# sevagh/umx.cpp

Hardware: AMD Instinct MI355X
Metric: realtime-factor (audio-sec/wall-sec) UMX-L 4-stem, 60 s seg (higher is better)
Workload: dtype f32 (activations as 2 x fp16 planes of the power-of-two-scaled row, integer weights exact in fp16, f32 accumulate on the fp16 matrix cores; fp32-grade: 1.4-2.2x the error of an fp32 evaluation, profiles/r06_v2_accuracy_vs_float64.txt)

## Files before the change

include/umx_hip.h:

```cpp
#ifndef UMX_HIP_H
#define UMX_HIP_H

#include <stddef.h>
#include <stdint.h>

#ifdef __cplusplus
extern "C" {
#endif

#define UMX_OK 0
#define UMX_ERR_ARG 1
#define UMX_ERR_HIP 2
#define UMX_ERR_MODEL 3
#define UMX_ERR_TIMEOUT 4
#define UMX_ERR_NODEVICE 5

#define UMX_DTYPE_F32 0
#define UMX_DTYPE_U8 1
#define UMX_DTYPE_U16 2

#define UMX_FLAG_NO_WIENER 0x1
#define UMX_FLAG_WIENER_ITERS_MASK 0xF0000u
#define UMX_FLAG_WIENER_ITERS(n) ((((unsigned)(n)) & 0xFu) << 16)
#define UMX_FLAG_SKIP_TARGET(t) (0x100 << (t))
// ... 187 lines not shown
    int n_out;
    int hop;
} umx_loudness;
int umx_hip_separate_tracks_loudness(umx_hip_ctx *ctx, int n_tracks, const void *const *audio_host, const int *length, const int *rate,
                                     const int *shift_offset, int n_out, const float *gains, void *const *out_host, unsigned flags,
                                     const umx_sample_io *io, int clip_mode, umx_levels *levels, umx_loudness *loudness,
                                     double *const *hop_energy, void (*progress)(float, void *), void *progress_user);
typedef void (*umx_queue_loudness_fn)(void *user, const umx_queue_job *job, const umx_levels *levels, const umx_loudness *loudness,
                                      const double *hop_energy);
int umx_hip_separate_queue_loudness(umx_hip_ctx *ctx, umx_queue_next_fn next, umx_queue_loudness_fn done, void *user, int n_out,
                                    const float *gains, unsigned flags, const umx_sample_io *io, int clip_mode);
int umx_hip_kweight_hops_device(umx_hip_ctx *ctx, int n_buffers, const float *const *in_dev, int n, int rate, long long first_hop,
                                long long n_hops, double *E_dev, void *hip_stream);
int umx_hip_kweight_coeffs(int rate, double pb[3], double pa[3], double rb[3], double ra[3]);
int umx_hip_kweight_hops_host(const float *x, int n, int rate, long long first_hop, long long n_hops, double *E);
int umx_hip_loudness_gate(const double *E, long long hops, int hop, double *integrated, double *momentary_max, long long *blocks,
                          long long *gated);
#define UMX_TRUE_PEAK_OFF 0
#define UMX_TRUE_PEAK_MEASURE 1
#define UMX_TRUE_PEAK_RESCALE 2
typedef struct umx_true_peak
{
    float true_peak[4];
    int n_out;
    int factor;
} umx_true_peak;
int umx_hip_separate_tracks_true_peak(umx_hip_ctx *ctx, int n_tracks, const void *const *audio_host, const int *length, const int *rate,
                                      const int *shift_offset, int n_out, const float *gains, void *const *out_host, unsigned flags,
                                      const umx_sample_io *io, int clip_mode, umx_levels *levels, umx_loudness *loudness,
                                      double *const *hop_energy, int true_peak_mode, umx_true_peak *true_peak,
                                      void (*progress)(float, void *), void *progress_user);
typedef void (*umx_queue_true_peak_fn)(void *user, const umx_queue_job *job, const umx_levels *levels, const umx_loudness *loudness,
                                       const double *hop_energy, const umx_true_peak *true_peak);
int umx_hip_separate_queue_true_peak(umx_hip_ctx *ctx, umx_queue_next_fn next, umx_queue_true_peak_fn done, void *user, int n_out,
                                     const float *gains, unsigned flags, const umx_sample_io *io, int clip_mode, int true_peak_mode);
int umx_hip_true_peak_device(umx_hip_ctx *ctx, int n_buffers, const float *const *in_dev, int n, int rate, long long first_frame,
                             long long n_frames, unsigned *bits_dev, void *hip_stream);
int umx_hip_true_peak_taps(int rate, float taps[49], int *factor);
int umx_hip_true_peak_host(const float *x, int n, int rate, long long first_frame, long long n_frames, unsigned *bits);
int umx_hip_debug_resample_taps(int rate_in, int rate_out, float *taps, size_t cap, int *phases, int *taps_per_phase,
                                int *first_offset);

size_t umx_hip_stream_layer_floats(const umx_hip_ctx *ctx);
int umx_hip_stream_get_layer(umx_hip_ctx *ctx, int layer, float *host_dst);
int umx_hip_stream_set_layer(umx_hip_ctx *ctx, int layer, const float *host_src);
int umx_hip_segment_begin(umx_hip_ctx *ctx, const float *audio_host, int n, unsigned flags);
int umx_hip_segment_lstm_layer(umx_hip_ctx *ctx, int layer);
int umx_hip_segment_end(umx_hip_ctx *ctx, float *const out_host[4]);

int umx_hip_segment_masks_device(umx_hip_ctx *ctx);
int umx_hip_segment_residual_device(umx_hip_ctx *ctx);
float *umx_hip_target_mag_device(umx_hip_ctx *ctx, int target, size_t *floats);
int umx_hip_segment_finish_device(umx_hip_ctx *ctx, float *const out_dev[4]);
int umx_hip_segment_discard(umx_hip_ctx *ctx);
int umx_hip_gate_reserve(int device, int cus);
void *umx_hip_phase_stream(umx_hip_ctx *ctx);
float *umx_hip_stream_state_device(umx_hip_ctx *ctx);
int umx_hip_segment_begin_device(umx_hip_ctx *ctx, const float *audio_dev, int n, unsigned flags);
int umx_hip_segment_end_device(umx_hip_ctx *ctx, float *const out_dev[4]);
int umx_hip_weight_stems_device(umx_hip_ctx *ctx, float *const stems_dev[4], int n, void *hip_stream);
int umx_hip_track_accumulate_device(umx_hip_ctx *ctx, float *const track_dev[4], float *sum_weight_dev,
                                    const float *const weighted_dev[4], int offset, int n, void *hip_stream);
int umx_hip_track_normalise_device(umx_hip_ctx *ctx, float *const track_dev[4], const float *sum_weight_dev, int length,
                                   void *hip_stream);

int umx_hip_nb_frames(const umx_hip_ctx *ctx);
int umx_hip_segment_samples(const umx_hip_ctx *ctx);
int umx_hip_hidden(const umx_hip_ctx *ctx);

long umx_hip_read_tap(umx_hip_ctx *ctx, const char *what, int target, float *dst, size_t capacity_floats);

int umx_hip_stage_times(umx_hip_ctx *ctx, const char **names, float *ms, int cap);
int umx_hip_stage_times_slot(umx_hip_ctx *ctx, int slot_index, const char **names, float *ms, int cap);
int umx_hip_stage_kernel_times_slot(umx_hip_ctx *ctx, int slot_index, float *ms, int cap);
int umx_hip_lstm_was_persistent(const umx_hip_ctx *ctx);
const char *umx_hip_lstm_kernel_name(const umx_hip_ctx *ctx);
const char *umx_hip_gemm_kernel_name(const umx_hip_ctx *ctx, int mode);
int umx_hip_lstm_mode(umx_hip_ctx *ctx);
int umx_hip_debug_wiener_bins(int n, const float *X, const float *masks, const float *R, float max_abs, float *y);
int umx_hip_debug_gate_math(int n, const float *x, float *fn, int n_waves, const float *pre, const float *c, float *cell);
int umx_hip_debug_lstm_profile(umx_hip_ctx *ctx, unsigned long long *out48);
int umx_hip_debug_lstm_placement(umx_hip_ctx *ctx, unsigned long long *out, int n);
int umx_hip_debug_lds_guard(umx_hip_ctx *ctx, int launches, int rounds, unsigned *out2);
unsigned umx_hip_debug_f16_bits(float x);
int umx_hip_debug_quant_centre(float scale, float offset, float *o2);
int umx_hip_debug_quant_planes(const void *q, int elem_size, int n, float scale, float offset, unsigned short *hi, unsigned short *lo, float *o2);

#ifdef __cplusplus
}
#endif
#endif
```

umx.cpp_amd/__init__.py:

```python
import ctypes as C
import os
import subprocess
from pathlib import Path

import numpy as np

from . import ggml

HERE = Path(__file__).resolve().parent
ROOT = HERE.parent
NB, CROP, KX, NOUT, NFFT, HOP = 2049, 1487, 2976, 4098, 4096, 1024
SEGMENT_SAMPLES = 60 * 44100

UMX_OK, ERR_ARG, ERR_HIP, ERR_MODEL, ERR_TIMEOUT, ERR_NODEVICE = 0, 1, 2, 3, 4, 5
HOST_ERR_AUDIO = 12
DTYPE_F32, DTYPE_U8, DTYPE_U16 = 0, 1, 2
FLAG_NO_WIENER = 0x1
FLAG_SOFTMASK = 0x2
FLAG_LSTM_STEPWISE = 0x10
FLAG_DEBUG_TAPS = 0x20
FLAG_LSTM_FORCE_SAFE = 0x40
FLAG_LSTM_PROFILE = 0x80
FLAG_PRECISE_ACT = 0x1000
FLAG_DEBUG_LSTM_ABORT = 0x2000
# ... 138 lines not shown
        import torch
        torch.cuda.is_available()
    except Exception:
        pass
    path = Path(os.environ.get("UMX_HIP_LIB", HERE / "libumx_hip.so"))
    if not path.exists():
        raise ImportError(f"{path} is missing: run `python -c 'import __graft_entry__ as g; g.build()'` "
                          "(hipcc --offload-arch=gfx950). There is no CPU fallback.")
    lib = C.CDLL(str(path))
    lib.umx_hip_create.argtypes = [C.POINTER(C.c_void_p), C.c_int, C.c_int, C.c_int, C.POINTER(TensorView), C.c_int]
    lib.umx_hip_create_ex.argtypes = [C.POINTER(C.c_void_p), C.c_int, C.c_int, C.c_int, C.POINTER(TensorView), C.c_int,
                                      C.c_uint]
    lib.umx_hip_create_tracks.argtypes = [C.POINTER(C.c_void_p), C.c_int, C.c_int, C.c_int, C.POINTER(TensorView), C.c_int,
                                          C.c_uint, C.c_int]
    lib.umx_hip_n_tracks.argtypes = [C.c_void_p]
    lib.umx_hip_pipeline_depth.argtypes = [C.c_void_p]
    lib.umx_hip_lstm_is_batched.argtypes = [C.c_void_p]
    lib.umx_hip_debug_f16_bits.argtypes = [C.c_float]
    lib.umx_hip_debug_f16_bits.restype = C.c_uint
    lib.umx_hip_debug_quant_centre.argtypes = [C.c_float, C.c_float, C.POINTER(C.c_float)]
    lib.umx_hip_debug_quant_centre.restype = C.c_int
    lib.umx_hip_debug_quant_planes.argtypes = [C.c_void_p, C.c_int, C.c_int, C.c_float, C.c_float, C.c_void_p, C.c_void_p, C.POINTER(C.c_float)]
    lib.umx_hip_debug_quant_planes.restype = C.c_int
    lib.umx_hip_track_stream_reset.argtypes = [C.c_void_p, C.c_int]
    lib.umx_hip_track_stream_get.argtypes = [C.c_void_p, C.c_int, _fp]
    lib.umx_hip_track_stream_set.argtypes = [C.c_void_p, C.c_int, _fp]
    lib.umx_hip_infer_segment_async.argtypes = [C.c_void_p, C.c_void_p, C.c_int, C.POINTER(C.c_void_p), C.c_uint]
    lib.umx_hip_infer_batch.argtypes = [C.c_void_p, C.c_int, C.POINTER(C.c_void_p), C.POINTER(C.c_int), C.POINTER(C.c_void_p), C.c_uint]
    lib.umx_hip_infer_batch_async.argtypes = lib.umx_hip_infer_batch.argtypes
    lib.umx_hip_infer_batch_device.argtypes = lib.umx_hip_infer_batch.argtypes
    lib.umx_hip_order_after.argtypes = [C.c_void_p, C.c_void_p]
    lib.umx_hip_order_before.argtypes = [C.c_void_p, C.c_void_p]
    lib.umx_hip_weight_bytes.restype = C.c_size_t
    lib.umx_hip_weight_bytes.argtypes = [C.c_void_p]
    lib.umx_hip_destroy.argtypes = [C.c_void_p]
    lib.umx_hip_last_error.restype = C.c_char_p
    lib.umx_hip_last_error.argtypes = [C.c_void_p]
    lib.umx_hip_stream_floats.restype = C.c_size_t
    lib.umx_hip_stream_floats.argtypes = [C.c_void_p]
    lib.umx_hip_stream_reset.argtypes = [C.c_void_p]
    lib.umx_hip_stream_get.argtypes = [C.c_void_p, _fp]
    lib.umx_hip_stream_set.argtypes = [C.c_void_p, _fp]
    lib.umx_hip_infer_segment.argtypes = [C.c_void_p, _fp, C.c_int, C.POINTER(_fp), C.c_uint]
    lib.umx_hip_infer_segment_device.argtypes = [C.c_void_p, C.c_void_p, C.c_int, C.POINTER(C.c_void_p), C.c_uint]
    lib.umx_hip_sync.argtypes = [C.c_void_p]
    lib.umx_hip_stream_handle.restype = C.c_void_p
    lib.umx_hip_stream_handle.argtypes = [C.c_void_p]
    lib.umx_hip_nb_frames.argtypes = [C.c_void_p]
    lib.umx_hip_segment_samples.argtypes = [C.c_void_p]
    lib.umx_hip_hidden.argtypes = [C.c_void_p]
    lib.umx_hip_read_tap.restype = C.c_long
    lib.umx_hip_read_tap.argtypes = [C.c_void_p, C.c_char_p, C.c_int, _fp, C.c_size_t]
    lib.umx_hip_stage_times.argtypes = [C.c_void_p, C.POINTER(C.c_char_p), _fp, C.c_int]
    lib.umx_hip_stage_times_slot.argtypes = [C.c_void_p, C.c_int, C.POINTER(C.c_char_p), _fp, C.c_int]
    lib.umx_hip_stage_kernel_times_slot.argtypes = [C.c_void_p, C.c_int, _fp, C.c_int]
    lib.umx_hip_lstm_was_persistent.argtypes = [C.c_void_p]
    lib.umx_hip_lstm_mode.argtypes = [C.c_void_p]
    lib.umx_hip_debug_lstm_profile.argtypes = [C.c_void_p, C.POINTER(C.c_ulonglong)]
    lib.umx_hip_debug_wiener_bins.argtypes = [C.c_int, _fp, _fp, _fp, C.c_float, _fp]
    lib.umx_hip_debug_gate_math.argtypes = [C.c_int, _fp, _fp, C.c_int, _fp, _fp, _fp]
    lib.umx_hip_lstm_kernel_name.restype = C.c_char_p
    lib.umx_hip_lstm_kernel_name.argtypes = [C.c_void_p]
    lib.umx_hip_gemm_kernel_name.restype = C.c_char_p
    lib.umx_hip_gemm_kernel_name.argtypes = [C.c_void_p, C.c_int]
    lib.umx_hip_debug_lstm_placement.argtypes = [C.c_void_p, C.POINTER(C.c_ulonglong), C.c_int]
    lib.umx_hip_stream_layer_floats.restype = C.c_size_t
    lib.umx_hip_stream_layer_floats.argtypes = [C.c_void_p]
    lib.umx_hip_stream_get_layer.argtypes = [C.c_void_p, C.c_int, _fp]
    lib.umx_hip_stream_set_layer.argtypes = [C.c_void_p, C.c_int, _fp]
    lib.umx_hip_segment_begin.argtypes = [C.c_void_p, _fp, C.c_int, C.c_uint]
    lib.umx_hip_segment_lstm_layer.argtypes = [C.c_void_p, C.c_int]
    lib.umx_hip_segment_end.argtypes = [C.c_void_p, C.POINTER(_fp)]
    lib.umx_hip_segment_begin_device.argtypes = [C.c_void_p, C.c_void_p, C.c_int, C.c_uint]
    lib.umx_hip_segment_end_device.argtypes = [C.c_void_p, C.POINTER(C.c_void_p)]
    lib.umx_hip_segment_masks_device.argtypes = [C.c_void_p]
    lib.umx_hip_segment_residual_device.argtypes = [C.c_void_p]
    lib.umx_hip_residual_slot.argtypes = [C.c_uint]
    lib.umx_hip_segment_finish_device.argtypes = [C.c_void_p, C.POINTER(C.c_void_p)]
    lib.umx_hip_weight_stems_device.argtypes = [C.c_void_p, C.POINTER(C.c_void_p), C.c_int, C.c_void_p]
    lib.umx_hip_track_accumulate_device.argtypes = [C.c_void_p, C.POINTER(C.c_void_p), C.c_void_p, C.POINTER(C.c_void_p), C.c_int,
                                                    C.c_int, C.c_void_p]
    lib.umx_hip_track_normalise_device.argtypes = [C.c_void_p, C.POINTER(C.c_void_p), C.c_void_p, C.c_int, C.c_void_p]
    lib.umx_hip_debug_lds_guard.argtypes = [C.c_void_p, C.c_int, C.c_int, C.POINTER(C.c_uint)]
    lib.umx_hip_split_inference.argtypes = [C.c_void_p, _fp, C.c_int, C.POINTER(_fp), C.c_uint, C.c_void_p, C.c_void_p]
    lib.umx_hip_shift_inference.argtypes = [C.c_void_p, _fp, C.c_int, C.c_int, C.POINTER(_fp), C.c_uint, C.c_void_p,
                                            C.c_void_p]
    lib.umx_hip_resampled_length.restype = C.c_longlong
    lib.umx_hip_resampled_length.argtypes = [C.c_longlong, C.c_int, C.c_int]
    lib.umx_hip_resample_device.argtypes = [C.c_void_p, C.c_int, C.c_int, C.c_int, C.POINTER(C.c_void_p), C.c_int,
                                            C.POINTER(C.c_void_p), C.c_int, C.c_void_p]
    lib.umx_hip_resample_needs.restype = C.c_longlong
    lib.umx_hip_resample_needs.argtypes = [C.c_longlong, C.c_int, C.c_int, C.c_longlong]
    lib.umx_hip_resample_ready.restype = C.c_longlong
    lib.umx_hip_resample_ready.argtypes = [C.c_longlong, C.c_int, C.c_int, C.c_longlong, C.c_longlong]
    lib.umx_hip_resample_range_device.argtypes = [C.c_void_p, C.c_int, C.c_int, C.c_int, C.POINTER(C.c_void_p), C.c_int,
                                                  C.POINTER(C.c_void_p), C.c_int, C.c_int, C.c_int, C.c_void_p]
    lib.umx_hip_debug_resample_launches.argtypes = [C.c_void_p, C.POINTER(C.c_int), C.POINTER(C.c_int)]
    lib.umx_hip_shift_inference_rate.argtypes = [C.c_void_p, _fp, C.c_int, C.c_int, C.c_int, C.POINTER(_fp), C.c_uint, C.c_void_p,
                                                 C.c_void_p]
    lib.umx_hip_debug_resample_taps.argtypes = [C.c_int, C.c_int, _fp, C.c_size_t, C.POINTER(C.c_int), C.POINTER(C.c_int),
                                                C.POINTER(C.c_int)]
    lib.umx_hip_ensemble_offsets.argtypes = [C.c_int, C.c_int, C.POINTER(C.c_int)]
    lib.umx_hip_shift_ensemble.argtypes = [C.c_void_p, _fp, C.c_int, C.c_int, C.c_int, C.POINTER(C.c_int), C.POINTER(_fp), C.c_uint,
                                           C.c_void_p, C.c_void_p]
    lib.umx_hip_debug_shift_mean_ms.restype = C.c_float
    lib.umx_hip_debug_shift_mean_ms.argtypes = [C.c_void_p]
    lib.umx_hip_mix_columns.argtypes = [C.c_int, _fp]
    lib.umx_hip_shift_ensemble_mix.argtypes = [C.c_void_p, _fp, C.c_int, C.c_int, C.c_int, C.POINTER(C.c_int), C.c_int, _fp, C.POINTER(_fp),
                                               C.c_uint, C.c_void_p, C.c_void_p]
    lib.umx_hip_mix_stems_device.argtypes = [C.c_void_p, C.c_int, _fp, C.POINTER(C.c_void_p), C.c_void_p, C.c_int, C.POINTER(C.c_void_p),
                                             C.c_void_p]
    lib.umx_hip_queue_plan.argtypes = [C.c_int, C.c_int, C.POINTER(C.c_int), C.POINTER(C.c_int), C.POINTER(C.c_int), C.POINTER(C.c_int)]
    lib.umx_hip_debug_queue_calls.argtypes = [C.c_void_p]
    lib.umx_hip_pcm16_decode_device.argtypes = [C.c_void_p, C.c_void_p, C.c_int, C.c_void_p, C.c_void_p]
    lib.umx_hip_pcm16_encode_device.argtypes = [C.c_void_p, C.c_int, C.POINTER(C.c_void_p), C.c_int, C.c_longlong, C.POINTER(SampleIO),
                                                C.POINTER(C.c_void_p), C.c_void_p]
    lib.umx_hip_pcm16_decode_host.argtypes = [_i16p, C.c_longlong, _fp]
    lib.umx_hip_pcm16_encode_host.argtypes = [_fp, C.c_int, C.c_int, C.c_longlong, C.POINTER(SampleIO), _i16p]
    lib.umx_hip_pcm24_decode_device.argtypes = [C.c_void_p, C.c_void_p, C.c_int, C.c_void_p, C.c_void_p]
    lib.umx_hip_pcm24_encode_device.argtypes = [C.c_void_p, C.c_int, C.POINTER(C.c_void_p), C.c_int, C.c_longlong, C.POINTER(SampleIO),
                                                C.POINTER(C.c_void_p), C.c_void_p]
    lib.umx_hip_pcm24_encode_rescaled_device.argtypes = [C.c_void_p, C.c_int, C.POINTER(C.c_void_p), C.c_int, C.c_longlong, C.POINTER(SampleIO),
                                                         C.POINTER(C.c_void_p), C.c_void_p, C.c_void_p]
    lib.umx_hip_pcm24_decode_host.argtypes = [_u8p, C.c_longlong, _fp]
    lib.umx_hip_pcm24_encode_host.argtypes = [_fp, C.c_int, C.c_int, C.c_longlong, C.POINTER(SampleIO), _u8p]
    lib.umx_hip_levels_device.argtypes = [C.c_void_p, C.c_int, C.POINTER(C.c_void_p), C.c_int, C.c_longlong, C.POINTER(SampleIO), C.c_void_p,
                                          C.c_void_p]
    lib.umx_hip_pcm16_encode_rescaled_device.argtypes = [C.c_void_p, C.c_int, C.POINTER(C.c_void_p), C.c_int, C.c_longlong, C.POINTER(SampleIO),
                                                         C.POINTER(C.c_void_p), C.c_void_p, C.c_void_p]
    lib.umx_hip_rescale_device.argtypes = [C.c_void_p, C.c_int, C.POINTER(C.c_void_p), C.c_int, C.c_void_p, C.c_void_p]
    lib.umx_hip_levels_host.argtypes = [_fp, C.c_int, C.c_int, C.c_longlong, C.POINTER(SampleIO), C.c_float, C.POINTER(LevelsAcc)]
    lib.umx_hip_rescale_gain.argtypes = [_fp, C.c_int]
    lib.umx_hip_rescale_gain.restype = C.c_float
    lib.umx_hip_kweight_hops_device.argtypes = [C.c_void_p, C.c_int, C.POINTER(C.c_void_p), C.c_int, C.c_int, C.c_longlong, C.c_longlong,
                                                C.c_void_p, C.c_void_p]
    lib.umx_hip_kweight_coeffs.argtypes = [C.c_int, _dp, _dp, _dp, _dp]
    lib.umx_hip_kweight_hops_host.argtypes = [_fp, C.c_int, C.c_int, C.c_longlong, C.c_longlong, _dp]
    lib.umx_hip_loudness_gate.argtypes = [_dp, C.c_longlong, C.c_int, _dp, _dp, C.POINTER(C.c_longlong), C.POINTER(C.c_longlong)]
    lib.umx_hip_true_peak_device.argtypes = [C.c_void_p, C.c_int, C.POINTER(C.c_void_p), C.c_int, C.c_int, C.c_longlong, C.c_longlong,
                                             C.c_void_p, C.c_void_p]
    lib.umx_hip_true_peak_taps.argtypes = [C.c_int, _fp, C.POINTER(C.c_int)]
    lib.umx_hip_true_peak_host.argtypes = [_fp, C.c_int, C.c_int, C.c_longlong, C.c_longlong, _up]
    def tracks_args(ptr, rate=True, mix=True):
        return ([C.c_void_p, C.c_int, C.POINTER(ptr), C.POINTER(C.c_int)] + [C.POINTER(C.c_int)] * (2 if rate else 1)
                + ([C.c_int, _fp] if mix else []) + [C.POINTER(ptr), C.c_uint])

    progress = [C.c_void_p, C.c_void_p]
    wide = tracks_args(C.c_void_p) + [C.POINTER(SampleIO)]
    lib.umx_hip_separate_tracks.argtypes = tracks_args(_fp, rate=False, mix=False) + progress
    lib.umx_hip_separate_tracks_rate.argtypes = tracks_args(_fp, mix=False) + progress
    lib.umx_hip_separate_tracks_mix.argtypes = tracks_args(_fp) + progress
    lib.umx_hip_separate_tracks_io.argtypes = wide + progress
    lib.umx_hip_separate_tracks_levels.argtypes = wide + [C.c_int, C.POINTER(Levels)] + progress
    lib.umx_hip_separate_tracks_loudness.argtypes = wide + [C.c_int, C.POINTER(Levels), C.POINTER(Loudness), C.POINTER(C.c_void_p)] + progress
    lib.umx_hip_separate_tracks_true_peak.argtypes = (wide + [C.c_int, C.POINTER(Levels), C.POINTER(Loudness), C.POINTER(C.c_void_p), C.c_int,
                                                              C.POINTER(TruePeak)] + progress)

    def queue_args(done_fn):
        return [C.c_void_p, QUEUE_NEXT_FN, done_fn, C.c_void_p, C.c_int, _fp, C.c_uint]

    lib.umx_hip_separate_queue.argtypes = queue_args(QUEUE_DONE_FN)
    lib.umx_hip_separate_queue_io.argtypes = queue_args(QUEUE_DONE_FN) + [C.POINTER(SampleIO)]
    lib.umx_hip_separate_queue_levels.argtypes = queue_args(QUEUE_LEVELS_FN) + [C.POINTER(SampleIO), C.c_int]
    lib.umx_hip_separate_queue_loudness.argtypes = queue_args(QUEUE_LOUDNESS_FN) + [C.POINTER(SampleIO), C.c_int]
    lib.umx_hip_separate_queue_true_peak.argtypes = queue_args(QUEUE_TRUE_PEAK_FN) + [C.POINTER(SampleIO), C.c_int, C.c_int]
    _hip = lib
    return lib


CREATE_QUANTISED_RESIDENT = 0x1
CREATE_GEMM_F32 = 0x4
CREATE_DEQUANTISE_AT_LOAD = 0x8
CREATE_LSTM_BATCHED = 0x10
CREATE_U8_DEQUANT = 0x20
CREATE_GEMM_STAGED = 0x40
CREATE_GEMM_PLANES = 0x80
MAX_TRACKS = 64
MAX_SHIFTS = MAX_TRACKS
MAX_MIX_OUTPUTS, MIX_COLUMNS, MIX_COLUMN_MIXTURE = 4, 5, 4
MODEL_RATE = 44100
RESAMPLE_MIN_RATE, RESAMPLE_MAX_RATE = 8000, 192000

HIP_SYMBOLS = ["umx_hip_create", "umx_hip_create_ex", "umx_hip_create_tracks", "umx_hip_n_tracks", "umx_hip_lstm_is_batched",
               "umx_hip_track_stream_reset", "umx_hip_track_stream_get", "umx_hip_track_stream_set",
               "umx_hip_infer_segment_async", "umx_hip_infer_batch", "umx_hip_infer_batch_async",
               "umx_hip_infer_batch_device", "umx_hip_order_after", "umx_hip_order_before",
               "umx_hip_separate_tracks", "umx_hip_phase_stream", "umx_hip_stream_state_device", "umx_hip_segment_begin_device", "umx_hip_segment_end_device",
               "umx_hip_weight_stems_device", "umx_hip_track_accumulate_device", "umx_hip_track_normalise_device", "umx_hip_weight_bytes", "umx_hip_destroy", "umx_hip_last_error", "umx_hip_stream_floats",
               "umx_hip_stream_reset", "umx_hip_stream_get", "umx_hip_stream_set", "umx_hip_infer_segment",
               "umx_hip_infer_segment_device", "umx_hip_sync", "umx_hip_stream_handle", "umx_hip_nb_frames",
               "umx_hip_segment_samples", "umx_hip_hidden", "umx_hip_read_tap", "umx_hip_stage_times",
               "umx_hip_stage_times_slot", "umx_hip_stage_kernel_times_slot",
               "umx_hip_lstm_was_persistent", "umx_hip_lstm_mode", "umx_hip_lstm_kernel_name", "umx_hip_gemm_kernel_name", "umx_hip_debug_wiener_bins", "umx_hip_debug_gate_math", "umx_hip_debug_lstm_profile", "umx_hip_debug_lstm_placement",
               "umx_hip_stream_layer_floats", "umx_hip_stream_get_layer", "umx_hip_stream_set_layer",
               "umx_hip_segment_begin", "umx_hip_segment_lstm_layer", "umx_hip_segment_end",
               "umx_hip_split_inference", "umx_hip_shift_inference", "umx_hip_debug_lds_guard", "umx_hip_debug_f16_bits", "umx_hip_debug_quant_centre", "umx_hip_debug_quant_planes",
               "umx_hip_segment_masks_device", "umx_hip_target_mag_device", "umx_hip_segment_finish_device", "umx_hip_gate_reserve", "umx_hip_segment_discard", "umx_hip_pipeline_depth",
               "umx_hip_resampled_length", "umx_hip_resample_device", "umx_hip_shift_inference_rate", "umx_hip_separate_tracks_rate",
               "umx_hip_debug_resample_taps", "umx_hip_residual_slot", "umx_hip_segment_residual_device",
               "umx_hip_ensemble_offsets", "umx_hip_shift_ensemble", "umx_hip_debug_shift_mean_ms",
               "umx_hip_mix_columns", "umx_hip_separate_tracks_mix", "umx_hip_shift_ensemble_mix", "umx_hip_mix_stems_device",
               "umx_hip_separate_queue", "umx_hip_queue_plan", "umx_hip_debug_queue_calls",
               "umx_hip_separate_tracks_io", "umx_hip_separate_queue_io", "umx_hip_pcm16_decode_device", "umx_hip_pcm16_encode_device",
               "umx_hip_pcm16_decode_host", "umx_hip_pcm16_encode_host",
               "umx_hip_separate_tracks_levels", "umx_hip_separate_queue_levels", "umx_hip_levels_device",
               "umx_hip_pcm16_encode_rescaled_device", "umx_hip_rescale_device", "umx_hip_levels_host", "umx_hip_rescale_gain",
               "umx_hip_separate_tracks_loudness", "umx_hip_separate_queue_loudness", "umx_hip_kweight_hops_device",
               "umx_hip_kweight_coeffs", "umx_hip_kweight_hops_host", "umx_hip_loudness_gate",
               "umx_hip_resample_needs", "umx_hip_resample_ready", "umx_hip_resample_range_device", "umx_hip_debug_resample_launches",
               "umx_hip_pcm24_decode_device", "umx_hip_pcm24_encode_device", "umx_hip_pcm24_encode_rescaled_device",
               "umx_hip_pcm24_decode_host", "umx_hip_pcm24_encode_host",
               "umx_hip_separate_tracks_true_peak", "umx_hip_separate_queue_true_peak", "umx_hip_true_peak_device",
               "umx_hip_true_peak_taps", "umx_hip_true_peak_host"]


def sample_io(in_format=SAMPLE_F32, out_format=SAMPLE_F32, dither_seed=None):
    return SampleIO(int(in_format), int(out_format), 0 if dither_seed is None else 1, 0 if dither_seed is None else int(dither_seed) & 0xFFFFFFFF)


def pcm16_decode_host(q):
    q = np.ascontiguousarray(q, np.int16)
    x = np.empty(q.shape, np.float32)
    rc = hip_lib().umx_hip_pcm16_decode_host(q.ctypes.data_as(_i16p), q.size, x.ctypes.data_as(_fp))
    if rc != UMX_OK:
        raise UmxError(rc, "umx_hip_pcm16_decode_host")
    return x


def _encode_host(fmt, x, buffer, first_frame, dither_seed):
    a = np.ascontiguousarray(np.asarray(x, np.float32).T)
    q, qp, out_format = {16: (np.empty(a.shape, np.int16), _i16p, SAMPLE_S16), 24: (np.empty(6 * a.shape[0], np.uint8), _u8p, SAMPLE_S24)}[fmt]
    io = sample_io(SAMPLE_F32, out_format, dither_seed)
    name = f"umx_hip_pcm{fmt}_encode_host"
    rc = getattr(hip_lib(), name)(a.ctypes.data_as(_fp), a.shape[0], int(buffer), int(first_frame), C.byref(io), q.ctypes.data_as(qp))
    if rc != UMX_OK:
        raise UmxError(rc, name)
    return q


def pcm16_encode_host(x, buffer=0, first_frame=0, dither_seed=None):
    return np.ascontiguousarray(_encode_host(16, x, buffer, first_frame, dither_seed).T)


def pcm24_pack(q):
    a = np.ascontiguousarray(np.asarray(q, np.int32).T)
    if a.ndim != 2 or a.shape[1] != 2:
        raise ValueError("pcm24_pack: need a (2, L) array")
    if a.size and (a.min() < -8388608 or a.max() > 8388607):
        raise ValueError("pcm24_pack: codes outside -8388608 .. 8388607")
    return np.ascontiguousarray(a.astype("<i4").view(np.uint8).reshape(-1, 4)[:, :3]).ravel()


def pcm24_unpack(b):
    b = np.ascontiguousarray(b, np.uint8).ravel()
    if b.size % 6:
        raise ValueError("pcm24_unpack: need a multiple of 6 bytes")
    w = np.zeros((b.size // 3, 4), np.uint8)
    w[:, 1:] = b.reshape(-1, 3)
    return np.ascontiguousarray((w.view("<i4").ravel().astype(np.int32) >> 8).reshape(-1, 2).T)


def pcm24_decode_host(q):
    q = np.ascontiguousarray(q, np.int32)
    b = np.ascontiguousarray(q.ravel().astype("<i4").view(np.uint8).reshape(-1, 4)[:, :3]).ravel()
    x = np.empty(q.shape, np.float32)
    rc = hip_lib().umx_hip_pcm24_decode_host(b.ctypes.data_as(_u8p), q.size, x.ctypes.data_as(_fp))
    if rc != UMX_OK:
        raise UmxError(rc, "umx_hip_pcm24_decode_host")
    return x


def pcm24_encode_host(x, buffer=0, first_frame=0, dither_seed=None):
    return pcm24_unpack(_encode_host(24, x, buffer, first_frame, dither_seed))


def levels_host(x, buffer=0, first_frame=0, io=None, clip_divisor=1.0, acc=None):
    a = np.ascontiguousarray(np.asarray(x, np.float32).T)
    acc = LevelsAcc() if acc is None else acc
    rc = hip_lib().umx_hip_levels_host(a.ctypes.data_as(_fp), a.shape[0], int(buffer), int(first_frame), None if io is None else C.byref(io),
# ... 647 lines not shown
            a = np.ascontiguousarray(wv.T).ravel()
            o = [np.empty(2 * wv.shape[1], np.float32) for _ in range(4)]
            keep.append((a, o))
            aud[i], ns[i] = a.ctypes.data, wv.shape[1]
            for t in range(4):
                outs[4 * i + t] = o[t].ctypes.data
        self._check(self.lib.umx_hip_infer_batch(self.h, nb, aud, ns, outs, flags))
        res, k = [], 0
        for wv in waves:
            if wv is None:
                res.append(None)
                continue
            n = keep[k][0].size // 2
            res.append([np.ascontiguousarray(o.reshape(n, 2).T) for o in keep[k][1]])
            k += 1
        return res

    def infer_batch_ptrs(self, audio_ptrs, ns, out_ptrs, flags=0, where="device"):
        nb = len(audio_ptrs)
        aud = (C.c_void_p * nb)(*[p or None for p in audio_ptrs])
        n_ = (C.c_int * nb)(*ns)
        outs = (C.c_void_p * (4 * nb))(*[p or None for p in out_ptrs])
        fn = self.lib.umx_hip_infer_batch_device if where == "device" else self.lib.umx_hip_infer_batch_async
        self._check(fn(self.h, nb, aud, n_, outs, flags))

    def infer_segment_device(self, audio_ptr, n, out_ptrs, flags=0):
        arr = (C.c_void_p * 4)(*out_ptrs)
        self._check(self.lib.umx_hip_infer_segment_device(self.h, C.c_void_p(audio_ptr), n, arr, flags))

    def sync(self):
        self._check(self.lib.umx_hip_sync(self.h))

    def last_error(self):
        return self.lib.umx_hip_last_error(self.h).decode()

    def lstm_was_persistent(self):
        return bool(self.lib.umx_hip_lstm_was_persistent(self.h))

    def lstm_mode(self):
        return self.lib.umx_hip_lstm_mode(self.h)

    def lstm_profile(self):
        buf = (C.c_ulonglong * 48)()
        self._check(self.lib.umx_hip_debug_lstm_profile(self.h, buf))
        a = np.array(buf[:], dtype=np.uint64).reshape(3, 2, 8)
        return a

    def gemm_kernel_name(self, mode):
        return self.lib.umx_hip_gemm_kernel_name(self.h, mode).decode()

    def lstm_kernel_name(self):
        return self.lib.umx_hip_lstm_kernel_name(self.h).decode()

    def lstm_placement(self, n=256):
        buf = (C.c_ulonglong * n)()
        self._check(self.lib.umx_hip_debug_lstm_placement(self.h, buf, n))
        a = np.array(buf[:], dtype=np.uint64)
        return [(int(v >> 48) & 15, int(v >> 40) & 255, int(v >> 32) & 255, int(v) & 0xffffffff) for v in a]

    def tap(self, what, target=0):
        n = self.lib.umx_hip_read_tap(self.h, what.encode(), target, None, 0)
        if n < 0:
            raise UmxError(ERR_ARG, f"tap {what!r} unavailable ({n})")
        buf = np.empty(n, np.float32)
        got = self.lib.umx_hip_read_tap(self.h, what.encode(), target, buf.ctypes.data_as(_fp), n)
        if got != n:
            raise UmxError(ERR_HIP, f"tap {what!r} failed ({got})")
        T, H = self.T, self.hidden
        what = what.split("@")[0].split("#")[0]
        if what in ("lstm_l0", "lstm_l1"):
            return buf.reshape(T, H)
        if what == "proj":
            return buf.reshape(T, 4 * H)
        if what in ("spec", "y"):
            return buf.view(np.complex64).reshape(2, T, NB)
        if what in ("mix_mag", "target_mag"):
            return buf.reshape(2, T, NB)
        if what == "x":
            return buf.reshape(T, KX)
        if what in ("fc1", "lstm", "fc2"):
            return buf.reshape(T, H)
        if what == "mask":
            return buf.reshape(T, NOUT)
        return buf

    def stage_times(self, slot=None):
        names = (C.c_char_p * 32)()
        ms = (C.c_float * 32)()
        if slot is None:
            n = self.lib.umx_hip_stage_times(self.h, names, ms, 32)
        else:
            n = self.lib.umx_hip_stage_times_slot(self.h, slot, names, ms, 32)
        return {names[i].decode(): float(ms[i]) for i in range(n)}

    def stage_kernel_times(self, slot=None):
        names = (C.c_char_p * 32)()
        ms = (C.c_float * 32)()
        n = self.lib.umx_hip_stage_times_slot(self.h, 0, names, (C.c_float * 32)(), 32)
        m = self.lib.umx_hip_stage_kernel_times_slot(self.h, -1 if slot is None else slot, ms, 32)
        return {names[i].decode(): float(ms[i]) for i in range(min(n, m))}


HOST_SYMBOLS = ["umx_model_load", "umx_model_free", "umx_model_hidden", "umx_model_n_tensors", "umx_model_views",
                "umx_model_data_bytes", "umx_model_load_progress", "umx_model_dequantize", "umx_wav_load",
                "umx_wav_free", "umx_wav_write_f32", "umx_wav_load_rate", "umx_wav_write_f32_rate",
                "umx_wav_load_pcm16", "umx_wav_free_pcm16", "umx_wav_write_pcm16_rate",
                "umx_wav_load_pcm24", "umx_wav_free_pcm24", "umx_wav_write_pcm24_rate", "umx_split_inference", "umx_shift_inference",
                "umx_segment_plan", "umx_transition_weight", "umx_split_inference_carry", "umx_split_inference_targets", "umx_mix_parse"]

SEGMENT_FN = C.CFUNCTYPE(C.c_int, C.c_void_p, _fp, C.c_int, C.POINTER(_fp))
RESET_FN = C.CFUNCTYPE(C.c_int, C.c_void_p)
PROGRESS_FN = C.CFUNCTYPE(None, C.c_float, C.c_void_p)


PH_BEGIN_FN = C.CFUNCTYPE(C.c_int, C.c_void_p, _fp, C.c_int)
PH_LAYER_FN = C.CFUNCTYPE(C.c_int, C.c_void_p, C.c_int)
PH_END_FN = C.CFUNCTYPE(C.c_int, C.c_void_p, C.POINTER(_fp))
PH_STATE_FN = C.CFUNCTYPE(C.c_int, C.c_void_p, C.c_int, _fp)
P2P_FN = C.CFUNCTYPE(C.c_int, C.c_void_p, _fp, C.c_size_t, C.c_int)


class PhasedBackend(C.Structure):
    _fields_ = [("begin", PH_BEGIN_FN), ("layer", PH_LAYER_FN), ("end", PH_END_FN), ("get_layer", PH_STATE_FN),
                ("set_layer", PH_STATE_FN), ("layer_floats", C.c_size_t), ("user", C.c_void_p)]


TG_BEGIN_FN = C.CFUNCTYPE(C.c_int, C.c_void_p, _fp, C.c_int, C.c_uint)
TG_STATE_FN = C.CFUNCTYPE(C.c_int, C.c_void_p, C.c_int, C.c_int, _fp)
TG_VOID_FN = C.CFUNCTYPE(C.c_int, C.c_void_p)
TG_MAG_FN = C.CFUNCTYPE(C.c_int, C.c_void_p, C.c_int, _fp)


class TargetBackend(C.Structure):
    _fields_ = [("begin", TG_BEGIN_FN), ("layer", PH_LAYER_FN), ("get_state", TG_STATE_FN), ("set_state", TG_STATE_FN),
                ("masks", TG_VOID_FN), ("get_mag", TG_MAG_FN), ("set_mag", TG_MAG_FN), ("finish", PH_END_FN), ("discard", TG_VOID_FN),
                ("target_layer_floats", C.c_size_t), ("mag_floats", C.c_size_t), ("user", C.c_void_p)]


class P2P(C.Structure):
    _fields_ = [("send", P2P_FN), ("recv", P2P_FN), ("user", C.c_void_p)]


class Backend(C.Structure):
    _fields_ = [("segment", SEGMENT_FN), ("reset", RESET_FN), ("user", C.c_void_p)]


_host = None


def host_lib():
    global _host
    if _host is not None:
        return _host
    path = HERE / "libumx_host.so"
    if not path.exists():
        raise ImportError(f"{path} is missing: run __graft_entry__.build()")
    lib = C.CDLL(str(path))
    lib.umx_model_load.argtypes = [C.c_char_p, C.POINTER(C.c_void_p), C.c_char_p]
    lib.umx_model_free.argtypes = [C.c_void_p]
    lib.umx_model_hidden.argtypes = [C.c_void_p]
    lib.umx_model_n_tensors.argtypes = [C.c_void_p]
    lib.umx_model_views.restype = C.POINTER(TensorView)
    lib.umx_model_views.argtypes = [C.c_void_p]
    lib.umx_model_data_bytes.restype = C.c_size_t
    lib.umx_model_data_bytes.argtypes = [C.c_void_p]
    lib.umx_model_load_progress.restype = C.c_float
    lib.umx_model_load_progress.argtypes = [C.c_void_p]
# ... 312 lines not shown
```

umx.cpp_amd/csrc/engine.hip:

```cpp
#include "../../include/umx_hip.h"
#include <chrono>
#include <dlfcn.h>

#include <algorithm>
#include <numeric>
#include <cmath>
#include <cstdio>
#include <cstdlib>
#include <cstring>
#include <map>
#include <mutex>
#include <string>
#include <vector>

#include "common.h"
#include "gemm_bf16x3.h"
#include "gemm_planes.h"
#include "gemm_planes_pp.h"
#include "gemm_planes_ps.h"
#include "lstm_kernels.h"
#include "lstm_batch.h"
#include "lstm_batch8.h"
#include "track_kernels.h"
#include "resample.h"
#include "stft_kernels.h"
#include "wiener_kernels.h"
#include "wiener_istft.h"
#include "wiener_em.h"
#include "residual_mask.h"
#include "softmask.h"
#include "shift_mean.h"
#include "stem_mix.h"
#include "sample_format.h"
#include "pcm16.h"
#include "pcm24.h"
#include "levels.h"
#include "loudness.h"
#include "true_peak.h"
#include "gate_debug.h"

using namespace umx;

#define UMX_HIP_CHECK_CTX(ctx_, expr)                                                                                \
    do                                                                                                               \
    {                                                                                                                \
        hipError_t _e = (expr);                                                                                      \
        if (_e != hipSuccess)                                                                                        \
        {                                                                                                            \
            (ctx_)->set_error(std::string(#expr) + ": " + hipGetErrorString(_e));                                    \
            return UMX_ERR_HIP;                                                                                      \
        }                                                                                                            \
    } while (0)

namespace
{
std::string g_create_error = "";

enum { W_FC1 = 0, W_IH0, W_IH1, W_IH2, W_FC2, W_FC3, W_COUNT };
inline int gemm_weight(int mode, int layer) { return mode == G_FC1 ? W_FC1 : mode == G_IH ? W_IH0 + layer : mode == G_FC2 ? W_FC2 : W_FC3; }

struct GemmWeight
{
    const void *p = nullptr;
    int form = 0;
    float s[2] = {1.f, 1.f}, o[2] = {0.f, 0.f};
    float c[2] = {128.f, 128.f}, o2[2] = {0.f, 0.f};
};

struct TargetBufs
{
    GemmWeight w[W_COUNT];
    float *in_scale = nullptr, *in_mean = nullptr, *bn1[4] = {};
    float *ih_b[3] = {};
    float *bn2[4] = {};
    float *bn3[4] = {}, *out_scale = nullptr, *out_mean = nullptr;
};

struct TargetAct
{
    float *cat = nullptr, *la = nullptr, *lb = nullptr, *P = nullptr, *a2 = nullptr,
          *mag = nullptr;
    unsigned short *xs_p = nullptr, *cat_p = nullptr, *la_p = nullptr, *lb_p = nullptr, *a2_p = nullptr;
    float *rs_xs = nullptr, *rs_catL = nullptr, *rs_catR = nullptr, *rs_la = nullptr, *rs_lb = nullptr, *rs_a2 = nullptr;
    float *rsc_xs = nullptr, *rsc_a2 = nullptr;
};

enum
{
    ST_STFT = 0,
    ST_FC1,
    ST_IH0,
    ST_LSTM0,
    ST_IH1,
    ST_LSTM1,
    ST_IH2,
    ST_LSTM2,
    ST_FC2,
    ST_FC3,
    ST_WIENER,
    ST_ISTFT,
    ST_OLA,
    ST_COUNT
};
enum { SP_XS = 0, SP_CATL, SP_LA, SP_LB, SP_CATR, SP_A2 };
const char *kStageNames[ST_COUNT] = {"stft",  "fc1", "lstm_ih0", "lstm_rec0", "lstm_ih1", "lstm_rec1", "lstm_ih2",
                                     "lstm_rec2", "fc2", "fc3_mask", "wiener",  "istft",    "ola"};

namespace
{
struct RoctxApi
{
    int (*push)(const char *) = nullptr;
    int (*pop)() = nullptr;
    char names[ST_COUNT][40];
    RoctxApi()
    {
        for (int i = 0; i < ST_COUNT; ++i)
            snprintf(names[i], sizeof names[i], "umx:%s", kStageNames[i]);
        const char *want = getenv("UMX_ROCTX");
        const bool force = want && atoi(want) != 0;
        for (const char *lib : {"librocprofiler-sdk-roctx.so", "libroctx64.so"})
            if (void *h = dlopen(lib, force ? (RTLD_NOW | RTLD_LOCAL) : (RTLD_NOW | RTLD_NOLOAD)))
            {
                push = reinterpret_cast<int (*)(const char *)>(dlsym(h, "roctxRangePushA"));
                pop = reinterpret_cast<int (*)()>(dlsym(h, "roctxRangePop"));
                if (push && pop)
                    return;
                push = nullptr;
                pop = nullptr;
            }
    }
};
thread_local bool t_stage_range_open = false;
inline void stage_range(int stage)
{
    static const RoctxApi api;
    if (!api.push)
        return;
    if (t_stage_range_open)
        api.pop();
    t_stage_range_open = stage >= 0 && stage < ST_COUNT;
    if (t_stage_range_open)
        api.push(api.names[stage]);
}
struct StageRangeCloser
{
    ~StageRangeCloser() { stage_range(-1); }
};
}

struct Lane
{
    TargetAct ta[4];
    float2 *spec = nullptr, *y = nullptr, *frames = nullptr;
    float *x = nullptr, *wpart = nullptr, *Rc = nullptr;
    unsigned *maxabs = nullptr;
};

// ... 577 lines not shown
```

umx.cpp_amd/csrc/engine_cabi.h:

```cpp
template <class From, class To>
static bool device_buffers(umx_hip_ctx *ctx, const char *what, int n_buffers, From *const *bufs, int n, long long first_frame, To *p[4])
{
    if (n_buffers < 1 || n_buffers > 4 || !bufs || n < 1 || first_frame < 0)
    {
        ctx->set_error(std::string(what) + ": need 1 .. 4 buffers, n >= 1 and first_frame >= 0");
        return false;
    }
    for (int b = 0; b < n_buffers; ++b)
    {
        if (!bufs[b])
        {
            ctx->set_error(std::string(what) + ": null buffer");
            return false;
        }
        p[b] = reinterpret_cast<To *>(bufs[b]);
    }
    return true;
}

struct DitherArg
{
    bool on;
    uint32_t seed;
};
// ... 902 lines not shown

__global__ void debug_wiener_bins_kernel(int n, const float *X, const float *masks, const float *R, float max_abs, float *y)
{
    const int b = blockIdx.x * blockDim.x + threadIdx.x;
    if (b >= n)
        return;
    const float2 X0 = make_float2(X[b * 4 + 0], X[b * 4 + 1]), X1 = make_float2(X[b * 4 + 2], X[b * 4 + 3]);
    const float h0 = mix_magnitude(X0), h1 = mix_magnitude(X1);
    float m0[4], m1[4];
    float4 rc[4];
    for (int s = 0; s < 4; ++s)
    {
        m0[s] = masks[(b * 4 + s) * 2 + 0] * h0;
        m1[s] = masks[(b * 4 + s) * 2 + 1] * h1;
        rc[s] = make_float4(R[(b * 4 + s) * 4 + 0], R[(b * 4 + s) * 4 + 1], R[(b * 4 + s) * 4 + 2], R[(b * 4 + s) * 4 + 3]);
    }
    WienerBin wb;
    wiener_bin_setup(X0, X1, m0, m1, rc, max_abs, 1.0f / max_abs, wb);
    for (int s = 0; s < 4; ++s)
    {
        float2 o[2];
        wiener_bin_apply(wb, s, rc[s], max_abs, o);
        y[((b * 4 + s) * 2 + 0) * 2 + 0] = o[0].x;
        y[((b * 4 + s) * 2 + 0) * 2 + 1] = o[0].y;
        y[((b * 4 + s) * 2 + 1) * 2 + 0] = o[1].x;
        y[((b * 4 + s) * 2 + 1) * 2 + 1] = o[1].y;
    }
}
int umx_hip_debug_wiener_bins(int n, const float *X, const float *masks, const float *R, float max_abs, float *y)
{
    if (n < 1 || !X || !masks || !R || !y || !(max_abs >= 1.0f))
        return UMX_ERR_ARG;
    float *d = nullptr;
    const size_t nx = (size_t)n * 4, nm = (size_t)n * 8, nr = (size_t)n * 16, ny = (size_t)n * 16;
    if (hipMalloc(reinterpret_cast<void **>(&d), (nx + nm + nr + ny) * sizeof(float)) != hipSuccess)
        return UMX_ERR_HIP;
    bool ok = hipMemcpy(d, X, nx * 4, hipMemcpyHostToDevice) == hipSuccess && hipMemcpy(d + nx, masks, nm * 4, hipMemcpyHostToDevice) == hipSuccess &&
              hipMemcpy(d + nx + nm, R, nr * 4, hipMemcpyHostToDevice) == hipSuccess;
    if (ok)
    {
        hipLaunchKernelGGL(debug_wiener_bins_kernel, dim3((n + 63) / 64), dim3(64), 0, nullptr, n, d, d + nx, d + nx + nm, max_abs, d + nx + nm + nr);
        ok = hipDeviceSynchronize() == hipSuccess && hipMemcpy(y, d + nx + nm + nr, ny * 4, hipMemcpyDeviceToHost) == hipSuccess;
    }
    (void)hipFree(d);
    return ok ? UMX_OK : UMX_ERR_HIP;
}

int umx_hip_debug_gate_math(int n, const float *x, float *fn, int n_waves, const float *pre, const float *c, float *cell)
{
    if (n < 0 || n_waves < 0 || (n > 0 && (!x || !fn)) || (n_waves > 0 && (!pre || !c || !cell)) || n > (1 << 24) || n_waves > (1 << 16))
        return UMX_ERR_ARG;
    const size_t nx = (size_t)n, nf = (size_t)5 * n, np_ = (size_t)n_waves * 64, nc = (size_t)n_waves * 16, no = (size_t)n_waves * 128;
    if (nx + np_ == 0)
        return UMX_OK;
    float *d = nullptr;
    if (hipMalloc(reinterpret_cast<void **>(&d), (nx + nf + np_ + nc + no) * sizeof(float)) != hipSuccess)
        return UMX_ERR_HIP;
    float *dx = d, *dfn = dx + nx, *dpre = dfn + nf, *dc = dpre + np_, *dcell = dc + nc;
    bool ok = true;
    if (n > 0)
    {
        ok = hipMemcpy(dx, x, nx * 4, hipMemcpyHostToDevice) == hipSuccess;
        if (ok)
            hipLaunchKernelGGL(debug_gate_fn_kernel, dim3((n + 255) / 256), dim3(256), 0, nullptr, n, dx, dfn);
    }
    if (ok && n_waves > 0)
    {
        ok = hipMemcpy(dpre, pre, np_ * 4, hipMemcpyHostToDevice) == hipSuccess && hipMemcpy(dc, c, nc * 4, hipMemcpyHostToDevice) == hipSuccess;
        if (ok)
        {
            hipLaunchKernelGGL(debug_gate_cell_kernel<0>, dim3(n_waves), dim3(64), 0, nullptr, dpre, dc, dcell);
            hipLaunchKernelGGL(debug_gate_cell_kernel<1>, dim3(n_waves), dim3(64), 0, nullptr, dpre, dc, dcell + nc * 2);
            hipLaunchKernelGGL(debug_gate_cell_kernel<2>, dim3(n_waves), dim3(64), 0, nullptr, dpre, dc, dcell + nc * 4);
            hipLaunchKernelGGL(debug_gate_cell_kernel<3>, dim3(n_waves), dim3(64), 0, nullptr, dpre, dc, dcell + nc * 6);
        }
    }
    ok = ok && hipDeviceSynchronize() == hipSuccess;
    if (ok && n > 0)
        ok = hipMemcpy(fn, dfn, nf * 4, hipMemcpyDeviceToHost) == hipSuccess;
    if (ok && n_waves > 0)
        ok = hipMemcpy(cell, dcell, no * 4, hipMemcpyDeviceToHost) == hipSuccess;
    (void)hipFree(d);
    return ok ? UMX_OK : UMX_ERR_HIP;
}

int umx_hip_debug_lds_guard(umx_hip_ctx *ctx, int launches, int rounds, unsigned *out2)
{
    static hipStream_t gs = nullptr;
    static unsigned *errs = nullptr;
    if (!ctx)
        return UMX_ERR_ARG;
    if (!gs)
    {
        if (hipStreamCreateWithFlags(&gs, hipStreamNonBlocking) != hipSuccess || hipMalloc(&errs, 8) != hipSuccess)
            return UMX_ERR_HIP;
        (void)hipMemset(errs, 0, 8);
    }
    for (int i = 0; i < launches; ++i)
        hipLaunchKernelGGL(lds_guard_kernel, dim3(512), dim3(256), 0, gs, errs, rounds);
    if (launches == 0 && out2)
    {
        (void)hipStreamSynchronize(gs);
        (void)hipMemcpy(out2, errs, 8, hipMemcpyDeviceToHost);
        (void)hipMemset(errs, 0, 8);
    }
    return UMX_OK;
}

int umx_hip_segment_begin(umx_hip_ctx *ctx, const float *audio_host, int n, unsigned flags)
{
    return ctx ? ctx->phase_begin(audio_host, n, flags) : UMX_ERR_ARG;
}
int umx_hip_segment_lstm_layer(umx_hip_ctx *ctx, int layer) { return ctx ? ctx->phase_layer(layer) : UMX_ERR_ARG; }
int umx_hip_segment_end(umx_hip_ctx *ctx, float *const out_host[4]) { return ctx ? ctx->phase_end(out_host) : UMX_ERR_ARG; }

void *umx_hip_phase_stream(umx_hip_ctx *ctx) { return ctx ? (void *)ctx->slot[0].stream : nullptr; }
float *umx_hip_stream_state_device(umx_hip_ctx *ctx) { return ctx ? ctx->state : nullptr; }
int umx_hip_segment_begin_device(umx_hip_ctx *ctx, const float *audio_dev, int n, unsigned flags)
{
    return ctx ? ctx->phase_begin_device(audio_dev, n, flags) : UMX_ERR_ARG;
}
int umx_hip_segment_end_device(umx_hip_ctx *ctx, float *const out_dev[4]) { return ctx ? ctx->phase_end_device(out_dev) : UMX_ERR_ARG; }
int umx_hip_segment_masks_device(umx_hip_ctx *ctx) { return ctx ? ctx->phase_masks() : UMX_ERR_ARG; }
int umx_hip_segment_residual_device(umx_hip_ctx *ctx) { return ctx ? ctx->phase_residual() : UMX_ERR_ARG; }
int umx_hip_residual_slot(unsigned flags) { return residual_slot_of(flags); }
int umx_hip_segment_discard(umx_hip_ctx *ctx)
{
    if (!ctx)
        return UMX_ERR_ARG;
    stage_range(-1);
    ctx->ph_next = -1;
    ctx->cur = 0;
    ctx->clear_used();
    return UMX_OK;
}
int umx_hip_segment_finish_device(umx_hip_ctx *ctx, float *const out_dev[4]) { return ctx ? ctx->phase_finish_device(out_dev) : UMX_ERR_ARG; }
float *umx_hip_target_mag_device(umx_hip_ctx *ctx, int target, size_t *floats)
{
    if (!ctx || target < 0 || target > 3)
        return nullptr;
    if (floats)
        *floats = (size_t)2 * ctx->T * MAGP;
    return ctx->slot[0].lane[0].ta[target].mag;
}
int umx_hip_gate_reserve(int device, int cus)
{
    if (device < 0)
        return UMX_ERR_ARG;
    LstmGate &g = g_gate[device & 15];
    std::lock_guard<std::mutex> lock(g.m);
    if (cus > 0)
        g.reservations.push_back(cus);
    else if (cus < 0)
    {
        auto it = std::find(g.reservations.begin(), g.reservations.end(), -cus);
        if (it == g.reservations.end())
            return UMX_ERR_ARG;
        g.reservations.erase(it);
    }
    else
        g.reservations.clear();
    g.reserved = 2 * std::accumulate(g.reservations.begin(), g.reservations.end(), 0);
    return UMX_OK;
}

static Stems4 stems4(float *const p[4])
// ... 197 lines not shown
    umx_hip_ctx::DeferredDownload d;
    d.valid = true;
    d.si = si;
    d.nb = n_tracks;
    for (int ln = 0; ln < n_tracks; ++ln)
    {
        d.n[ln] = ain[ln] ? n[ln] : 0;
        for (int s = 0; s < 4; ++s)
            d.host[4 * ln + s] = out_host[4 * ln + s];
    }
    return ctx->queue_download(d, ctx->copy_stream);
}

int umx_hip_infer_batch(umx_hip_ctx *ctx, int n_tracks, const float *const *audio_host, const int *n, float *const *out_host,
                        unsigned flags)
{
    if (int rc = umx_hip_infer_batch_async(ctx, n_tracks, audio_host, n, out_host, flags))
        return rc;
    return umx_hip_sync(ctx);
}

int umx_hip_infer_segment_async(umx_hip_ctx *ctx, const float *audio_host, int n, float *const out_host[4], unsigned flags)
{
    if (!ctx || !audio_host || !out_host)
    {
        if (ctx)
            ctx->set_error("infer_segment: bad arguments");
        return UMX_ERR_ARG;
    }
    return umx_hip_infer_batch_async(ctx, 1, &audio_host, &n, out_host, flags);
}

int umx_hip_infer_segment(umx_hip_ctx *ctx, const float *audio_host, int n, float *const out_host[4], unsigned flags)
{
    if (int rc = umx_hip_infer_segment_async(ctx, audio_host, n, out_host, flags))
        return rc;
    return umx_hip_sync(ctx);
}

void *umx_hip_stream_handle(umx_hip_ctx *ctx) { return ctx ? (void *)ctx->slot[ctx->cur].stream : nullptr; }
int umx_hip_nb_frames(const umx_hip_ctx *ctx) { return ctx ? ctx->T : 0; }
int umx_hip_segment_samples(const umx_hip_ctx *ctx) { return ctx ? ctx->N : 0; }
int umx_hip_hidden(const umx_hip_ctx *ctx) { return ctx ? ctx->H : 0; }

long umx_hip_read_tap(umx_hip_ctx *ctx, const char *what, int target, float *dst, size_t cap)
{
    if (!ctx || !what || target < 0 || target > 3)
        return -1;
    std::string w = what;
    const int T = ctx->T, H = ctx->H;
    int which = ctx->cur, lane = 0;
    {
        const size_t hash = w.find('#');
        if (hash != std::string::npos)
        {
            lane = atoi(w.c_str() + hash + 1);
            const size_t at = w.find('@', hash);
            w = w.substr(0, hash) + (at == std::string::npos ? "" : w.substr(at));
            if (lane < 0 || lane >= ctx->B)
                return -1;
        }
    }
    if (w.size() > 2 && w[w.size() - 2] == '@')
    {
        which = w.back() - '0';
        w = w.substr(0, w.size() - 2);
        if (which < 0 || which >= ctx->nslots)
            return -1;
    }
    const Lane &sl = ctx->slot[which].lane[lane];
    const void *src = nullptr;
    size_t nfl = 0, src_ld = 0, rows = 0, cols = 0;
    int computed = 0;
    if (w == "spec") { src = sl.spec; nfl = (size_t)2 * 2 * T * NBINS; }
    else if (w == "mix_mag") { src = sl.spec; computed = 1; nfl = (size_t)2 * T * NBINS; }
    else if (w == "x") { src = sl.x; nfl = (size_t)T * KX; }
    else if (w == "fc1") { src = sl.ta[target].cat; rows = T; cols = H; src_ld = 2 * H; nfl = rows * cols; }
    else if (w == "lstm") { src = sl.ta[target].cat + H; rows = T; cols = H; src_ld = 2 * H; nfl = rows * cols; }
    else if (w == "lstm_l0") { src = sl.ta[target].la; nfl = (size_t)T * H; }
    else if (w == "lstm_l1") { src = sl.ta[target].lb; nfl = (size_t)T * H; }
    else if (w == "proj") { src = sl.ta[target].P; nfl = (size_t)T * 4 * H; }
    else if (w == "fc2") { src = sl.ta[target].a2; nfl = (size_t)T * H; }
    else if (w == "mask") { src = sl.ta[target].mag; computed = 3; nfl = (size_t)T * NOUT; }
    else if (w == "target_mag") { src = sl.ta[target].mag; computed = 2; nfl = (size_t)2 * T * NBINS; }
    else if (w == "y") { src = sl.y + (size_t)target * 2 * T * NBINS; nfl = (size_t)2 * 2 * T * NBINS; }
    else if (w == "max_abs") { src = sl.maxabs; nfl = 1; }
    else return -1;
    if ((w == "lstm" && !ctx->slot[which].lstm_rows_f32[2]) || (w == "lstm_l0" && !ctx->slot[which].lstm_rows_f32[0]) ||
        (w == "lstm_l1" && !ctx->slot[which].lstm_rows_f32[1]))
        return -2;
    if (!src)
        return -2;
    if (!dst)
        return (long)nfl;
    if (cap < nfl)
        return -3;
    if (ctx->sync_all() != UMX_OK)
        return -4;
    if (computed)
    {
        if (!ctx->tap_tmp && ctx->dalloc(&ctx->tap_tmp, (size_t)2 * T * NBINS) != UMX_OK)
            return -4;
        const unsigned blocks = (unsigned)((nfl + 255) / 256);
        if (computed == 1)
            hipLaunchKernelGGL(tap_mix_mag_kernel, dim3(blocks), dim3(256), 0, nullptr, sl.spec, nfl, ctx->tap_tmp);
        else if (computed == 2)
            hipLaunchKernelGGL(tap_target_mag_kernel, dim3(blocks), dim3(256), 0, nullptr, sl.spec, sl.ta[target].mag, nfl, ctx->tap_tmp);
        else
            hipLaunchKernelGGL(tap_mask_kernel, dim3(blocks), dim3(256), 0, nullptr, sl.ta[target].mag, T, ctx->tap_tmp);
        if (hipDeviceSynchronize() != hipSuccess)
            return -4;
        src = ctx->tap_tmp;
    }
    hipError_t e;
    if (rows)
        e = hipMemcpy2D(dst, cols * sizeof(float), src, src_ld * sizeof(float), cols * sizeof(float), rows,
                        hipMemcpyDeviceToHost);
    else
        e = hipMemcpy(dst, src, nfl * sizeof(float), hipMemcpyDeviceToHost);
    if (e != hipSuccess)
    {
        ctx->set_error(hipGetErrorString(e));
        return -4;
    }
    if (w == "max_abs")
    {
        unsigned bits;
        memcpy(&bits, dst, 4);
        float m;
        memcpy(&m, &bits, 4);
        dst[0] = std::max(1.0f, m / WIENER_SCALE);
    }
    return (long)nfl;
}

int umx_hip_stage_times_slot(umx_hip_ctx *ctx, int slot_index, const char **names, float *ms, int cap);
int umx_hip_stage_times(umx_hip_ctx *ctx, const char **names, float *ms, int cap)
{
    return ctx ? umx_hip_stage_times_slot(ctx, ctx->cur, names, ms, cap) : 0;
}

int umx_hip_stage_times_slot(umx_hip_ctx *ctx, int slot_index, const char **names, float *ms, int cap)
{
    if (!ctx || slot_index < 0 || slot_index >= ctx->nslots)
        return 0;
    Slot &sl = ctx->slot[slot_index];
    if (!sl.have_times || ctx->sync_all() != UMX_OK)
        return 0;
    int n = std::min(cap, (int)ST_COUNT);
    for (int i = 0; i < n; ++i)
    {
        float t = 0.f;
        (void)hipEventElapsedTime(&t, sl.ev[i], sl.ev[i + 1]);
        if (names)
            names[i] = kStageNames[i];
        if (ms)
            ms[i] = t;
    }
    return ST_COUNT;
}

int umx_hip_stage_kernel_times_slot(umx_hip_ctx *ctx, int slot_index, float *ms, int cap)
{
    if (ctx && slot_index < 0)
        slot_index = ctx->cur;
    if (!ctx || slot_index >= ctx->nslots)
// ... 54 lines not shown
```

umx.cpp_amd/csrc/engine_init.h:

```cpp
namespace
{
bool dequant(const umx_tensor_view &tv, size_t expect, std::vector<float> &out)
{
    size_t nel = 1;
    for (int i = 0; i < tv.n_dims; ++i)
        nel *= (size_t)tv.ne[i];
    if (nel != expect)
        return false;
    out.resize(nel);
    if (tv.dtype == UMX_DTYPE_F32)
        memcpy(out.data(), tv.data, nel * sizeof(float));
    else if (tv.dtype == UMX_DTYPE_U8)
    {
        const uint8_t *q = static_cast<const uint8_t *>(tv.data);
        for (size_t i = 0; i < nel; ++i)
            out[i] = (float)q[i] * tv.scale + tv.offset;
    }
    else if (tv.dtype == UMX_DTYPE_U16)
    {
        const uint16_t *q = static_cast<const uint16_t *>(tv.data);
        for (size_t i = 0; i < nel; ++i)
            out[i] = (float)q[i] * tv.scale + tv.offset;
    }
    else
// ... 37 lines not shown
    device = device_;
    UMX_HIP_CHECK(hipSetDevice(device));
    H = hidden;
    Hl = H / 2;
    S = Hl / LSTM_UNITS_PER_WG;
    N = segment_samples;
    T = N / HOP + 1;
    Tp = T;
    nbatch = (T + WIENER_BATCH - 1) / WIENER_BATCH;

    std::map<std::string, const umx_tensor_view *> idx[4];
    for (int i = 0; i < n_tensors; ++i)
    {
        if (tensors[i].target < 0 || tensors[i].target > 3 || !tensors[i].name || !tensors[i].data)
        {
            set_error("tensor view with bad target / name / data");
            return UMX_ERR_MODEL;
        }
        idx[tensors[i].target][tensors[i].name] = &tensors[i];
    }
    auto get = [&](int tg, const std::string &name, size_t expect, std::vector<float> &out) -> bool {
        auto it = idx[tg].find(name);
        if (it == idx[tg].end())
        {
            set_error("missing tensor '" + name + "' for target " + std::to_string(tg));
            return false;
        }
        if (!dequant(*it->second, expect, out))
        {
            set_error("tensor '" + name + "' has wrong size in model (target " + std::to_string(tg) + ")");
            return false;
        }
        return true;
    };

    const bool keepq = !(create_flags & UMX_CREATE_DEQUANTISE_AT_LOAD);
    auto view = [&](int tg, const std::string &name) -> const umx_tensor_view * {
        auto it = idx[tg].find(name);
        return it == idx[tg].end() ? nullptr : it->second;
    };
    auto all_q = [&](const std::string &name, int dtype, size_t expect) {
        for (int tg = 0; tg < 4; ++tg)
        {
            const umx_tensor_view *tv = view(tg, name);
            size_t n = 1;
            for (int i = 0; tv && i < tv->n_dims; ++i)
                n *= (size_t)tv->ne[i];
            if (!keepq || !tv || tv->dtype != dtype || n != expect)
                return false;
        }
        return true;
    };

    if (create_flags & UMX_CREATE_GEMM_F32)
    {
        set_error("UMX_CREATE_GEMM_F32: the fp32-MFMA GEMM flavour was removed in round 3 (slower and, against float64, less accurate "
                  "than the split-operand kernels: profiles/r02_accuracy_vs_float64.txt)");
        return UMX_ERR_ARG;
    }
    if (const char *e = getenv("UMX_GEMM_PP"))
        env_gemm_pp = atoi(e);
    if (const char *e = getenv("UMX_GEMM_PS"))
        env_gemm_ps = atoi(e);
    if (const char *e = getenv("UMX_LSTM8_POLL_DELAY"))
        lstm8_poll_delay = atoi(e);
    if (const char *e = getenv("UMX_LSTM8_PAIRED"))
        env_lstm8_paired = atoi(e) != 0;
    if (const char *e = getenv("UMX_LSTM8_MIN_LANES"))
        env_lstm8_min = atoi(e);
    if (const char *e = getenv("UMX_LSTM_POLL_DELAY"))
        lstm_poll_delay = atoi(e);
    wiener_fused = lstm_batched;
    if (const char *e = getenv("UMX_WIENER"))
        wiener_fused = std::string(e) == "fused";
    gemm_planes = (create_flags & UMX_CREATE_GEMM_PLANES) || (lstm_batched && !(create_flags & UMX_CREATE_GEMM_STAGED));
    Tp = gemm_planes ? std::max(T, 256) : round_up(T, 128);

    const int G = 4 * Hl;
    std::vector<int> gate_row(G);
    for (int sl = 0; sl < S; ++sl)
        for (int g = 0; g < 4; ++g)
            for (int u = 0; u < 16; ++u)
                gate_row[g * Hl + sl * 16 + u] = sl * 64 + u * 4 + g;
    std::vector<int> fc3_row(NOUT);
    for (int r = 0; r < NOUT; ++r)
        fc3_row[r] = r / NBINS * MAGP + r % NBINS;
    struct WeightDesc
    {
        std::string name[2];
        int nsrc, rows, cols, dst_rows, cols_pad;
        const std::vector<int> *dst_row;
        int dtype;
    };
    WeightDesc wd[W_COUNT];
    wd[W_FC1] = {{"fc1.weight"}, 1, H, NIN, H, KX, nullptr, UMX_DTYPE_U8};
    for (int l = 0; l < 3; ++l)
        wd[W_IH0 + l] = {{"lstm.weight_ih_l" + std::to_string(l), "lstm.weight_ih_l" + std::to_string(l) + "_reverse"}, 2, G, H, G, H, &gate_row,
                         UMX_DTYPE_U8};
    wd[W_FC2] = {{"fc2.weight"}, 1, H, 2 * H, H, 2 * H, nullptr, UMX_DTYPE_U16};
    wd[W_FC3] = {{"fc3.weight"}, 1, NOUT, H, NOUT_PAD, H, &fc3_row, UMX_DTYPE_U16};
    auto upload_weight = [&](GemmWeight &w, const void *host, size_t bytes) -> int {
        unsigned char *p = nullptr;
        if (int rc = dalloc(&p, bytes, false))
            return rc;
        UMX_HIP_CHECK(hipMemcpy(p, host, bytes, hipMemcpyHostToDevice));
        w.p = p;
        weight_bytes += bytes;
        return UMX_OK;
    };
    const bool exact_ok = keepq && !u8_dequant;
    auto load_weight = [&](int tg, const WeightDesc &d, GemmWeight &w) -> int {
        const size_t n = (size_t)d.nsrc * d.dst_rows * d.cols_pad;
        auto dst = [&](int s, int r) { return ((size_t)s * d.dst_rows + (d.dst_row ? (*d.dst_row)[r] : r)) * d.cols_pad; };
        bool q = true;
        for (int s = 0; s < d.nsrc; ++s)
            q = q && all_q(d.name[s], d.dtype, (size_t)d.rows * d.cols);
        std::vector<unsigned short> planes;
        if (q && (!gemm_planes || exact_ok))
        {
            const size_t esz = d.dtype == UMX_DTYPE_U8 ? 1 : 2;
            if (gemm_planes)
            {
                w.form = (int)esz;
                planes.assign(w.form * n, 0);
                for (int s = 0; s < d.nsrc; ++s)
                {
                    const umx_tensor_view *tv = view(tg, d.name[s]);
                    unsigned short *hi = planes.data() + (size_t)s * d.dst_rows * d.cols_pad;
                    const QuantCentre qc = quant_planes(tv->data, (int)esz, d.rows, d.cols, d.dst_row ? d.dst_row->data() : nullptr, (size_t)d.cols_pad,
                                                        tv->scale, tv->offset, hi, esz == 2 ? hi + n : nullptr);
                    w.s[s] = tv->scale;
                    w.o[s] = qc.o2;
                }
                return upload_weight(w, planes.data(), planes.size() * sizeof(unsigned short));
            }
            std::vector<unsigned char> qh(n * esz, 0);
            for (int s = 0; s < d.nsrc; ++s)
            {
                const umx_tensor_view *tv = view(tg, d.name[s]);
                for (int r = 0; r < d.rows; ++r)
                    memcpy(&qh[dst(s, r) * esz], static_cast<const unsigned char *>(tv->data) + (size_t)r * d.cols * esz, (size_t)d.cols * esz);
                w.s[s] = tv->scale;
                w.o[s] = tv->offset;
            }
            for (int s = 0; s < d.nsrc && esz == 1; ++s)
            {
                const QuantCentre qc = quant_centre(w.s[s], w.o[s]);
                w.c[s] = (float)qc.c;
                w.o2[s] = qc.o2;
            }
            w.form = esz == 1 ? BQ_U8 : BQ_U16;
            return upload_weight(w, qh.data(), qh.size());
        }
        std::vector<float> f(n, 0.f), v;
        if (gemm_planes)
            planes.assign(2 * n, 0);
        for (int s = 0; s < d.nsrc; ++s)
        {
            if (!get(tg, d.name[s], (size_t)d.rows * d.cols, v))
                return UMX_ERR_MODEL;
            for (int r = 0; r < d.rows; ++r)
                memcpy(&f[dst(s, r)], &v[(size_t)r * d.cols], sizeof(float) * d.cols);
            if (gemm_planes)
            {
                float mx = 0.f, scale = 1.f;
                for (float x : v)
                    if (std::isfinite(x))
                        mx = std::max(mx, std::fabs(x));
                if (mx > 0.f)
                {
                    int x;
                    (void)std::frexp(mx, &x);
                    const int e = std::min(std::max(GP_SPLIT_FIXED_EXP + 1 - x, -100), 100);
                    scale = std::ldexp(1.0f, e);
                    w.s[s] = std::ldexp(1.0f, -e);
                }
                const size_t b0 = (size_t)s * d.dst_rows * d.cols_pad;
                for (size_t i = b0; i < b0 + (size_t)d.dst_rows * d.cols_pad; ++i)
                    f16_split(f[i] * scale, &planes[i], &planes[n + i]);
            }
        }
        if (gemm_planes)
            w.form = 2;
        else
        {
            w.form = BQ_F32;
            planes.resize(3 * n);
            for (size_t i = 0; i < n; ++i)
                split3_host(f[i], planes[i], planes[n + i], planes[2 * n + i]);
        }
        return upload_weight(w, planes.data(), planes.size() * sizeof(unsigned short));
    };

    std::vector<float> whh_h[3], bhh_h[3];
    std::vector<unsigned char> whh_qh[3];
    bool whh_all_u8 = true;
    for (int l = 0; l < 3; ++l)
        for (int dir = 0; dir < 2; ++dir)
            whh_all_u8 = whh_all_u8 && all_q("lstm.weight_hh_l" + std::to_string(l) + (dir ? "_reverse" : ""), UMX_DTYPE_U8, (size_t)G * Hl);
    if (whh_all_u8)
        for (int l = 0; l < 3; ++l)
            whh_qh[l].assign((size_t)8 * S * Hl * 64, 0);
    for (int l = 0; l < 3; ++l)
    {
        whh_h[l].assign((size_t)8 * S * Hl * 64, 0.f);
        bhh_h[l].assign((size_t)8 * S * 64, 0.f);
    }
    for (int tg = 0; tg < 4; ++tg)
    {
        TargetBufs &b = tb[tg];
        std::vector<float> v, w;
        if (!get(tg, "input_scale", CROP, v))
            return UMX_ERR_MODEL;
        w.assign(KX, 0.f);
        for (int k = 0; k < NIN; ++k)
            w[k] = v[k % CROP];
        if (int rc = upload(&b.in_scale, w))
            return rc;
        if (!get(tg, "input_mean", CROP, v))
            return UMX_ERR_MODEL;
        w.assign(KX, 0.f);
        for (int k = 0; k < NIN; ++k)
            w[k] = v[k % CROP];
        if (int rc = upload(&b.in_mean, w))
            return rc;
        if (!get(tg, "output_scale", NBINS, v))
            return UMX_ERR_MODEL;
        w.assign(NOUT_PAD, 0.f);
        for (int c = 0; c < 2; ++c)
            for (int k = 0; k < NBINS; ++k)
                w[c * MAGP + k] = v[k];
        if (int rc = upload(&b.out_scale, w))
            return rc;
        if (!get(tg, "output_mean", NBINS, v))
            return UMX_ERR_MODEL;
        w.assign(NOUT_PAD, 0.f);
        for (int c = 0; c < 2; ++c)
            for (int k = 0; k < NBINS; ++k)
                w[c * MAGP + k] = v[k];
        if (int rc = upload(&b.out_mean, w))
            return rc;
        if (int rc = load_weight(tg, wd[W_FC1], b.w[W_FC1]))
            return rc;
        const char *bnn[4] = {"running_mean", "running_var", "weight", "bias"};
        for (int k = 0; k < 4; ++k)
        {
            if (!get(tg, std::string("bn1.") + bnn[k], H, v))
                return UMX_ERR_MODEL;
            if (int rc = upload(&b.bn1[k], v))
                return rc;
            if (!get(tg, std::string("bn2.") + bnn[k], H, v))
                return UMX_ERR_MODEL;
            if (int rc = upload(&b.bn2[k], v))
                return rc;
            if (!get(tg, std::string("bn3.") + bnn[k], NOUT, v))
                return UMX_ERR_MODEL;
            w.assign(NOUT_PAD, k == 1 ? 1.f : 0.f);
            for (int c = 0; c < 2; ++c)
                memcpy(&w[c * MAGP], &v[c * NBINS], sizeof(float) * NBINS);
            if (int rc = upload(&b.bn3[k], w))
                return rc;
        }
        if (int rc = load_weight(tg, wd[W_FC2], b.w[W_FC2]))
            return rc;
        if (int rc = load_weight(tg, wd[W_FC3], b.w[W_FC3]))
            return rc;
        for (int l = 0; l < 3; ++l)
        {
            if (int rc = load_weight(tg, wd[W_IH0 + l], b.w[W_IH0 + l]))
                return rc;
            std::vector<float> ihb((size_t)2 * G);
            for (int dir = 0; dir < 2; ++dir)
            {
                const std::string sfx = "_l" + std::to_string(l) + (dir ? "_reverse" : "");
                std::vector<float> whhv, bih, bhhv;
                if ((!whh_all_u8 && !get(tg, "lstm.weight_hh" + sfx, (size_t)G * Hl, whhv)) ||
                    !get(tg, "lstm.bias_ih" + sfx, G, bih) || !get(tg, "lstm.bias_hh" + sfx, G, bhhv))
                    return UMX_ERR_MODEL;
                const int chain = tg * 2 + dir;
                const umx_tensor_view *hhv = view(tg, "lstm.weight_hh" + sfx);
                const unsigned char *hhq = whh_all_u8 ? static_cast<const unsigned char *>(hhv->data) : nullptr;
                if (whh_all_u8)
                {
                    whh_s[l][chain] = hhv->scale;
                    whh_o[l][chain] = hhv->offset;
                }
                for (int row = 0; row < G; ++row)
                {
                    const int sl = gate_row[row] / 64, col = gate_row[row] % 64;
                    ihb[(size_t)dir * G + gate_row[row]] = bih[row];
                    bhh_h[l][((size_t)chain * S + sl) * 64 + col] = bhhv[row];
                    for (int k = 0; k < Hl; ++k)
                    {
                        const size_t di = (((size_t)chain * S + sl) * Hl + k) * 64 + col;
                        if (whh_all_u8)
                            whh_qh[l][di] = hhq[(size_t)row * Hl + k];
                        else
                            whh_h[l][di] = whhv[(size_t)row * Hl + k];
                    }
                }
            }
            if (int rc = upload(&b.ih_b[l], ihb))
                return rc;
        }
    }
    for (int l = 0; l < 3; ++l)
    {
        if (whh_all_u8)
        {
            if (int rc = upload(&whh_q[l], whh_qh[l]))
                return rc;
            weight_bytes += whh_qh[l].size();
        }
        else
        {
            if (int rc = upload(&whh[l], whh_h[l]))
                return rc;
            weight_bytes += whh_h[l].size() * sizeof(float);
        }
        if (int rc = upload(&bhh[l], bhh_h[l]))
            return rc;
    }
    {
        std::vector<float> w(NFFT);
        static const float PI = 3.14159265359F;
        const float floatN = (float)(NFFT + 1);
        for (int n = 0; n < NFFT; ++n)
            w[n] = 0.5F * (1.0F - cosf(2.0F * PI * (float)n / (floatN - 1)));
        if (int rc = upload(&window, w))
            return rc;
        const size_t total = (size_t)NFFT + (size_t)HOP * (T - 1);
        std::vector<float> nwh(total, 0.f);
        for (int i = 0; i < T; ++i)
        {
            const size_t s0 = (size_t)i * HOP;
            for (size_t j = s0; j < std::min(total, s0 + NFFT); ++j)
                nwh[j] += w[j - s0] * w[j - s0];
        }
        if (int rc = upload(&nw, nwh))
            return rc;
        std::vector<float2> t1(256), t2(4096);
        for (int r = 0; r < 16; ++r)
            for (int k = 0; k < 16; ++k)
            {
// ... 254 lines not shown
```

umx.cpp_amd/csrc/engine_stages.h:

```cpp
void umx_hip_ctx::launch_gemm(Lane &sl, hipStream_t st, int mode, int layer, const int *active, int nact, bool dbg)
{
    GemmArgs g;
    memset(&g, 0, sizeof g);
    g.M = Tp;
    g.T = T;
    int bq = BQ_F32;
    for (int i = 0; i < nact; ++i)
    {
        const TargetBufs &b = tb[active[i]];
        const TargetAct &c = sl.ta[active[i]];
        const GemmWeight &w = b.w[gemm_weight(mode, layer)];
        GemmTarget &t = g.t[i];
        switch (mode)
        {
        case G_FC1:
            t.A = sl.x; t.C = c.cat;
            t.e0 = b.bn1[0]; t.e1 = b.bn1[1]; t.e2 = b.bn1[2]; t.e3 = b.bn1[3];
            t.q0 = b.in_scale; t.q1 = b.in_mean;
            g.N = H; g.K = KX; g.lda = KX; g.ldc = 2 * H;
            break;
        case G_IH:
            t.A = layer == 0 ? c.cat : layer == 1 ? c.la : c.lb;
            t.C = c.P; t.e0 = b.ih_b[layer];
            g.N = 4 * H; g.K = H; g.lda = layer == 0 ? 2 * H : H; g.ldc = 4 * H;
            break;
        case G_FC2:
            t.A = c.cat; t.C = c.a2;
            t.e0 = b.bn2[0]; t.e1 = b.bn2[1]; t.e2 = b.bn2[2]; t.e3 = b.bn2[3];
            g.N = H; g.K = 2 * H; g.lda = 2 * H; g.ldc = H;
            break;
        default:
            t.A = c.a2; t.C = c.mag;
            t.e0 = b.bn3[0]; t.e1 = b.bn3[1]; t.e2 = b.bn3[2]; t.e3 = b.bn3[3];
            t.q0 = b.out_scale; t.q1 = b.out_mean;
            g.N = NOUT_PAD; g.K = H; g.lda = H; g.ldc = 0;
            break;
        }
        t.Bq = w.p;
        t.bs[0] = w.s[0]; t.bs[1] = w.s[1];
        t.bo[0] = w.o[0]; t.bo[1] = w.o[1];
        t.bc[0] = w.c[0]; t.bc[1] = w.c[1];
        t.bo2[0] = w.o2[0]; t.bo2[1] = w.o2[1];
        t.bsplit = mode == G_IH ? 2 * H : 0x7fffffff;
        bq = w.form;
    }
    if (bq == BQ_U8 && !u8_dequant)
        bq = BQ_U8X;
    const GemmKernel k = bx_kernel(mode, bq);
    const dim3 grid((unsigned)round_up((g.N / GEMM_BN) * (g.M / GEMM_BM), 8), 1, nact), block(256);
    gemm_kernel_last[mode] = "gemm_bf16x3_kernel";
    void *kargs[] = {&g};
    (void)hipLaunchKernel(k.fn, grid, block, kargs, k.lds, st);
}

void umx_hip_ctx::launch_split(Lane &ln, int nl, hipStream_t st, int which, const int *active, int nact)
{
    SplitArgs a;
    memset(&a, 0, sizeof a);
    a.T = T;
    a.Tp = Tp;
    const size_t rows_all = (size_t)B * Tp + Mpad;
    for (int i = 0; i < nact; ++i)
    {
        const TargetBufs &b = tb[active[i]];
        const TargetAct &c = ln.ta[active[i]];
        switch (which)
        {
        case SP_XS:
            a.src[i] = ln.x; a.dst[i] = c.xs_p; a.rowsum[i] = c.rs_xs; a.rowunscale[i] = c.rsc_xs; a.scale[i] = b.in_scale; a.mean[i] = b.in_mean;
            a.cols = KX; a.ld_src = KX; a.ld_dst = KX; a.col0_dst = 0; a.plane = rows_all * KX;
            break;
        case SP_CATL:
            a.src[i] = c.cat; a.dst[i] = c.cat_p; a.rowsum[i] = c.rs_catL;
            a.cols = H; a.ld_src = 2 * H; a.ld_dst = 2 * H; a.col0_dst = 0; a.plane = rows_all * 2 * H;
            break;
        case SP_CATR:
            a.src[i] = c.cat + H; a.dst[i] = c.cat_p; a.rowsum[i] = lstm_rowsums ? nullptr : c.rs_catR;
            a.cols = H; a.ld_src = 2 * H; a.ld_dst = 2 * H; a.col0_dst = H; a.plane = rows_all * 2 * H;
            break;
        case SP_LA:
            a.src[i] = c.la; a.dst[i] = c.la_p; a.rowsum[i] = lstm_rowsums ? nullptr : c.rs_la;
            a.cols = H; a.ld_src = H; a.ld_dst = H; a.col0_dst = 0; a.plane = rows_all * H;
            break;
        case SP_LB:
            a.src[i] = c.lb; a.dst[i] = c.lb_p; a.rowsum[i] = lstm_rowsums ? nullptr : c.rs_lb;
            a.cols = H; a.ld_src = H; a.ld_dst = H; a.col0_dst = 0; a.plane = rows_all * H;
            break;
        default:
            a.src[i] = c.a2; a.dst[i] = c.a2_p; a.rowsum[i] = c.rs_a2; a.rowunscale[i] = c.rsc_a2;
            a.cols = H; a.ld_src = H; a.ld_dst = H; a.col0_dst = 0; a.plane = rows_all * H;
            break;
        }
    }
    a.rows_valid = nl * Tp;
    const dim3 grid(round_up(nl * Tp, 256) / 4, 1, nact);
    if (which == SP_XS && a.cols <= 3072)
    {
        hipLaunchKernelGGL(split_planes_shared_kernel<6>, dim3(grid.x), dim3(256), 0, st, a, nact);
        return;
    }
    if (a.cols <= 1024)
        hipLaunchKernelGGL(split_planes_kernel<2>, grid, dim3(256), 0, st, a);
    else if (a.cols <= 3072)
        hipLaunchKernelGGL(split_planes_kernel<6>, grid, dim3(256), 0, st, a);
    else
        hipLaunchKernelGGL(split_planes_kernel<8>, grid, dim3(256), 0, st, a);
}

void umx_hip_ctx::launch_gemm_planes(Lane &ln, int nl, hipStream_t st, int mode, int layer, const int *active, int nact, bool dbg)
{
    GemmPArgs g;
    memset(&g, 0, sizeof g);
    g.M = round_up(nl * Tp, 256);
    g.lanes = nl;
    g.T = T;
    g.Tp_lane = Tp;
    g.mag_lane = (size_t)2 * T * MAGP;
    g.a_unscale = 1.0f / (float)(1 << GP_SPLIT_FIXED_EXP);
    const size_t rows_all = (size_t)B * Tp + Mpad;
    int nbp = 2;
    for (int i = 0; i < nact; ++i)
    {
        const TargetBufs &b = tb[active[i]];
        const TargetAct &c = ln.ta[active[i]];
        const GemmWeight &w = b.w[gemm_weight(mode, layer)];
        GemmPTarget &t = g.t[i];
        t.bsplit = 0x7fffffff;
        switch (mode)
        {
        case G_FC1:
            t.A = c.xs_p; t.C = c.cat; t.rs0 = c.rs_xs; t.rsc = c.rsc_xs;
            t.e0 = b.bn1[0]; t.e1 = b.bn1[1]; t.e2 = b.bn1[2]; t.e3 = b.bn1[3];
            g.N = H; g.K = KX; g.lda = KX; g.ldc = 2 * H; g.a_plane = rows_all * KX;
            break;
        case G_IH:
            t.A = layer == 0 ? c.cat_p : layer == 1 ? c.la_p : c.lb_p;
            t.rs0 = layer == 0 ? c.rs_catL : layer == 1 ? c.rs_la : c.rs_lb;
            if (layer > 0 && lstm_rowsums)
                t.rs1 = t.rs0 + rows_all;
            t.C = c.P; t.e0 = b.ih_b[layer];
            t.bsplit = 2 * H;
            g.N = 4 * H; g.K = H; g.lda = layer == 0 ? 2 * H : H; g.ldc = 4 * H;
            g.a_plane = layer == 0 ? rows_all * 2 * H : rows_all * H;
            break;
        case G_FC2:
            t.A = c.cat_p; t.C = c.a2; t.rs0 = c.rs_catL; t.rs1 = c.rs_catR;
            if (lstm_rowsums)
                t.rs2 = c.rs_catR + rows_all;
            t.e0 = b.bn2[0]; t.e1 = b.bn2[1]; t.e2 = b.bn2[2]; t.e3 = b.bn2[3];
            g.N = H; g.K = 2 * H; g.lda = 2 * H; g.ldc = H; g.a_plane = rows_all * 2 * H;
            break;
        default:
            t.A = c.a2_p; t.C = c.mag; t.rs0 = c.rs_a2; t.rsc = c.rsc_a2;
            t.e0 = b.bn3[0]; t.e1 = b.bn3[1]; t.e2 = b.bn3[2]; t.e3 = b.bn3[3];
            t.q0 = b.out_scale; t.q1 = b.out_mean;
            g.N = NOUT_PAD; g.K = H; g.lda = H; g.ldc = 0; g.a_plane = rows_all * H;
            break;
        }
        t.B = static_cast<const unsigned short *>(w.p);
        t.bs[0] = w.s[0]; t.bs[1] = w.s[1];
        t.bo2[0] = w.o[0]; t.bo2[1] = w.o[1];
        nbp = w.form;
    }
    const int blocks_big = (g.N / 256) * (g.M / 256) * nact;
    const bool big = g.N % 256 == 0 && blocks_big >= 224;
    const int bm = big ? 256 : 128;
    const int gemm_pp = env_gemm_pp;
    const bool pp = big && (gemm_pp < 0 || ((gemm_pp >> mode) & 1));
    const int ps_wgs = n_cus / 8 * 8;
    const bool ps = pp && (env_gemm_ps < 0 || ((env_gemm_ps >> mode) & 1)) && g.K / GP_BK >= 6 && ps_wgs >= 8 && blocks_big > ps_wgs && g.Tp_lane >= 256;
    gemm_kernel_last[mode] = ps ? "gemm_planes_ps_kernel" : pp ? "gemm_planes_pp_kernel" : "gemm_planes_kernel";
    const GemmKernel k = gp_kernel(mode, nbp, ps ? GP_PS : pp ? GP_PP : big ? GP_256 : GP_128);
    void *kargs[] = {&g, &nact};
    if (ps)
        (void)hipLaunchKernel(k.fn, dim3(ps_wgs), dim3(512), kargs, k.lds, st);
    else
        (void)hipLaunchKernel(k.fn, dim3((unsigned)round_up((g.N / bm) * (g.M / bm), 8), 1, nact), dim3(pp ? 512 : big ? 1024 : 256), kargs,
                              k.lds, st);
}

void umx_hip_ctx::launch_gemm_lanes(Slot &sl, hipStream_t st, int nb, const float *const *audio_dev, int mode, int layer,
                                    const int *active, int nact, bool dbg)
{
    if (nact <= 0)
        return;
    for (int l0 = 0; l0 < nb;)
    {
        if (!audio_dev[l0])
        {
            ++l0;
            continue;
        }
        int l1 = l0 + 1;
        while (gemm_planes && l1 < nb && audio_dev[l1])
            ++l1;
        if (gemm_planes)
        {
            const int which = mode == G_FC1 ? SP_XS : mode == G_IH ? (layer == 0 ? SP_CATL : layer == 1 ? SP_LA : SP_LB) : mode == G_FC2 ? SP_CATR : SP_A2;
            const int from_layer = which == SP_LA ? 0 : which == SP_LB ? 1 : which == SP_CATR ? 2 : -1;
            if (from_layer < 0 || !sl.lstm_wrote_planes[from_layer])
                launch_split(sl.lane[l0], l1 - l0, st, which, active, nact);
            {
                const int stg = mode == G_FC1 ? ST_FC1 : mode == G_IH ? ST_IH0 + 2 * layer : mode == G_FC2 ? ST_FC2 : ST_FC3;
                sl.evk_set[stg] = sl.evk[stg] && hipEventRecord(sl.evk[stg], st) == hipSuccess;
            }
            launch_gemm_planes(sl.lane[l0], l1 - l0, st, mode, layer, active, nact, dbg);
        }
        else
            launch_gemm(sl.lane[l0], st, mode, layer, active, nact, dbg);
        l0 = l1;
    }
}

int umx_hip_ctx::stage_front(Slot &sl, hipStream_t st, int nb, const float *const *audio_dev, const int *n, const int *active,
                             int nact)
{
    stage_range(ST_STFT);
    for (int i = 0; i < ST_COUNT; ++i)
        sl.evk_set[i] = false;
    UMX_HIP_CHECK(hipEventRecord(sl.ev[ST_STFT], st));
    {
        StftIn in;
        in.lanes = lane_set(nb, audio_dev);
        for (int i = 0; i < in.lanes.count; ++i)
        {
            in.audio[i] = audio_dev[in.lanes.id[i]];
            in.n[i] = n[in.lanes.id[i]];
        }
        Lane &L0 = sl.lane[0];
        UMX_HIP_CHECK(hipMemsetAsync(L0.maxabs, 0, sizeof(unsigned) * B, st));
        hipLaunchKernelGGL(stft_kernel, dim3((T + STFT_RUN - 1) / STFT_RUN, in.lanes.count), dim3(256), 0, st, in, N, T, window, tw1, tw2, L0.spec, lane_strides().spec, L0.x,
                           (size_t)Tp * KX, L0.maxabs);
    }
    stage_range(ST_FC1);
    UMX_HIP_CHECK(hipEventRecord(sl.ev[ST_FC1], st));
    launch_gemm_lanes(sl, st, nb, audio_dev, G_FC1, 0, active, nact, false);
    stage_range(ST_IH0);
    UMX_HIP_CHECK(hipEventRecord(sl.ev[ST_IH0], st));
    launch_gemm_lanes(sl, st, nb, audio_dev, G_IH, 0, active, nact, false);
// ... 312 lines not shown
```

umx.cpp_amd/csrc/gemm_common.h:

```cpp
#pragma once
#include <cmath>
#include <type_traits>
#include "common.h"
#include "quant_planes.h"

namespace umx
{

typedef float floatx16 __attribute__((ext_vector_type(16)));

enum GemmMode
{
    G_FC1 = 0,
    G_IH = 1,
    G_FC2 = 2,
    G_FC3 = 3
};

struct GemmTarget
{
    const float *A;
    const float *B;
    float *C;
    const float *e0, *e1, *e2, *e3;
    const float *q0, *q1;
    const void *Bq;
    float bs[2], bo[2];
    float bc[2], bo2[2];
    int bsplit;
};


struct GemmArgs
{
    GemmTarget t[4];
    int M, N, K, lda, ldc, T;
    int Tp_lane, lanes;
    size_t mag_lane;
};

#ifndef GEMM_GROUP_M
#define GEMM_GROUP_M 8
#endif
constexpr int GEMM_BM = 128, GEMM_BN = 128;

__device__ __forceinline__ float4 scale_shift(float4 a, float4 sc, float4 mn)
{
    return make_float4(a.x * sc.x + mn.x, a.y * sc.y + mn.y, a.z * sc.z + mn.z, a.w * sc.w + mn.w);
}

__device__ __forceinline__ float tanh_epi(float x)
{
    const float ax = fabsf(x), u = x * x;
    const float e = __builtin_amdgcn_exp2f(ax * -2.88539008177792681f);
    const float big = (1.0f - e) * __builtin_amdgcn_rcpf(1.0f + e);
    float q = fmaf(u, -0.006946978159248829f, 0.021472707390785217f);
    q = fmaf(u, q, -0.05393378809094429f);
    q = fmaf(u, q, 0.1333322674036026f);
    q = fmaf(u, q, -0.3333333134651184f);
    const float small = ax * fmaf(u, q, 1.0f);
    return copysignf(ax < 0.5f ? small : big, x);
}

template <int MODE>
__device__ __forceinline__ void gemm_epilogue(const GemmTarget &tg, const GemmArgs &args, int m0, int n0, int wm, int wn,
                                              int lr, int lh, const floatx16 &acc00, const floatx16 &acc01,
                                              const floatx16 &acc10, const floatx16 &acc11)
{
    int f0 = m0;
    unsigned lo = 0;
    const int tpl = args.Tp_lane ? args.Tp_lane : (1 << 30);
    if (MODE == G_FC3 && args.Tp_lane)
    {
        const int ln = __builtin_amdgcn_readfirstlane(m0 / args.Tp_lane);
        f0 = m0 - ln * args.Tp_lane;
        lo = (unsigned)(ln * args.mag_lane);
    }
    const int m_next = tpl - f0;
    const int mlb = wm * 64 + 4 * lh;
    const int fA = f0 + mlb, fB = mlb - m_next;
    const unsigned dA = ((unsigned)args.mag_lane - (unsigned)args.Tp_lane * MAGP) * 4u;
    const int lanes = args.Tp_lane ? (args.lanes ? args.lanes : args.M / args.Tp_lane) : 1;
    const unsigned mag_bytes = MODE == G_FC3 ? (unsigned)((args.Tp_lane ? (size_t)lanes * args.mag_lane : (size_t)2 * args.T * MAGP) * 4) : 0u;
    const __amdgpu_buffer_rsrc_t rs_mag = __builtin_amdgcn_make_buffer_rsrc(tg.C, 0, mag_bytes, 0x00020000);
#pragma unroll
    for (int ni = 0; ni < 2; ++ni)
    {
        const int n = n0 + wn * 64 + ni * 32 + lr;
        float rm = 0.f, sd = 1.f, rsd = 1.f, gw = 1.f, gb = 0.f, osc = 1.f, omn = 0.f;
        if (MODE == G_IH)
            gb = tg.e0[n];
        else
        {
            rm = tg.e0[n];
            sd = sqrtf(tg.e1[n] + 1e-5f);
            rsd = 1.0f / sd;
            gw = tg.e2[n];
            gb = tg.e3[n];
        }
        unsigned col = (unsigned)n;
        bool col_ok = true;
        if (MODE == G_FC3)
        {
            osc = tg.q0[n];
            omn = tg.q1[n];
            const int c = n >= MAGP ? 1 : 0, bin = n - c * MAGP;
            col = lo + (unsigned)(c * args.T) * MAGP + (unsigned)bin;
            col_ok = bin < NBINS;
        }
        unsigned run = (col + (unsigned)fA * MAGP) * 4u;
        int frow = fB;
#pragma unroll
        for (int mi = 0; mi < 2; ++mi)
#pragma unroll
            for (int rq = 0; rq < 4; ++rq)
            {
                float ys[4];
                unsigned offs[4];
#pragma unroll
                for (int j = 0; j < 4; ++j)
                {
                    const int r = 4 * rq + j;
                    const int ml = wm * 64 + mi * 32 + j + 8 * rq + 4 * lh;
                    float y = mi == 0 ? (ni == 0 ? acc00[r] : acc01[r]) : (ni == 0 ? acc10[r] : acc11[r]);
                    if (MODE == G_IH)
                        tg.C[(size_t)(m0 + ml) * args.ldc + n] = y + gb;
                    else
                    {
                        y = div_by(y - rm, sd, rsd) * gw + gb;
                        if (MODE == G_FC1)
                            tg.C[(size_t)(m0 + ml) * args.ldc + n] = tanh_epi(y);
                        else if (MODE == G_FC2)
                            tg.C[(size_t)(m0 + ml) * args.ldc + n] = fmaxf(y, 0.f);
                        else
                        {
                            const bool second = frow >= 0;
                            const int f = second ? frow : frow + tpl;
                            const bool ok = col_ok && f < args.T;
                            ys[j] = fmaxf(y * osc + omn, 0.f);
                            offs[j] = ok ? run + (second ? dA : 0u) : 0xfffffff0u;
                            run += MAGP * 4;
                            frow += 1;
                        }
                    }
                }
                if (MODE == G_FC3)
                {
#pragma unroll
                    for (int j = 0; j < 4; ++j)
                        __builtin_amdgcn_raw_buffer_store_b32(__float_as_uint(ys[j]), rs_mag, offs[j], 0, 0);
                    run += 4 * MAGP * 4;
                    frow += 4;
                }
                asm volatile("" ::: "memory");
                __builtin_amdgcn_sched_barrier(0);
            }
    }
}

enum GemmBType
{
    BQ_F32 = 0,
    BQ_U8 = 1,
    BQ_U16 = 2,
    BQ_U8X = 3
};

__device__ __forceinline__ float4 deq_u8x4(unsigned p, float sc, float of)
{
    return make_float4((float)(p & 255u) * sc + of, (float)((p >> 8) & 255u) * sc + of,
                       (float)((p >> 16) & 255u) * sc + of, (float)(p >> 24) * sc + of);
}
__device__ __forceinline__ float4 deq_u16x4(uint2 p, float sc, float of)
{
    return make_float4((float)(p.x & 65535u) * sc + of, (float)(p.x >> 16) * sc + of,
                       (float)(p.y & 65535u) * sc + of, (float)(p.y >> 16) * sc + of);
}


}
```

umx.cpp_amd/csrc/gemm_planes.h:

```cpp
#pragma once
#include "gemm_bf16x3.h"
#include <cmath>
#include <cstring>

namespace umx
{

struct GemmPTarget
{
    const unsigned short *A;
    const unsigned short *B;
    float *C;
    const float *e0, *e1, *e2, *e3, *q0, *q1;
    const float *rs0, *rs1, *rs2;
    const float *rsc;
    float bs[2], bo2[2];
    int bsplit;
};

struct GemmPArgs
{
    GemmPTarget t[4];
    int M, N, K, lda, ldc, T;
    size_t a_plane;
    float a_unscale;
    int Tp_lane;
    int lanes;
    size_t mag_lane;
};

constexpr int GP_BK = 32;
constexpr int GP_SPLIT_FIXED_EXP = 14;
__host__ __device__ constexpr int gp_stage_bytes(int WM, int WN, int NBP) { return (2 * 64 * WM + NBP * 64 * WN) * 64; }
__host__ __device__ constexpr int gp_stages(int WM, int WN, int NBP)
{
    return 3 * gp_stage_bytes(WM, WN, NBP) <= (WM * WN >= 16 ? 160 : 80) * 1024 ? 3 : 2;
}
__host__ __device__ constexpr int gp_lds_bytes(int WM, int WN, int NBP) { return gp_stages(WM, WN, NBP) * gp_stage_bytes(WM, WN, NBP); }


struct SplitArgs
{
    const float *src[4];
    unsigned short *dst[4];
    float *rowsum[4];
    float *rowunscale[4];
    const float *scale[4], *mean[4];
    int T, Tp, cols, ld_src, ld_dst, col0_dst;
    int rows_valid;
    size_t plane;
};

typedef _Float16 f16x8 __attribute__((ext_vector_type(8)));

#ifndef GP_MFMA_K32
#define GP_MFMA_K32 1
#endif
typedef float floatx4 __attribute__((ext_vector_type(4)));
__device__ __forceinline__ int gp_k32_frag_offset(int lane)
{
    const int q = lane >> 4, c = (q + 3) & 3;
    return (lane & 15) * 64 + (c ^ ((lane >> 2) & 3)) * 16;
}
__device__ __forceinline__ void gp_k32_to_square(floatx4 &x, floatx4 &y)
{
#pragma unroll
    for (int j = 0; j < 4; ++j)
    {
        auto s = __builtin_amdgcn_permlane16_swap(__float_as_uint(x[j]), __float_as_uint(y[j]), false, false);
        s = __builtin_amdgcn_permlane32_swap(s[0], s[1], false, false);
        x[j] = __uint_as_float(s[0]);
        y[j] = __uint_as_float(s[1]);
    }
}
template <int MI> __device__ __forceinline__ void gp_k32_to_squares(const floatx4 (&acc4)[2 * MI][4], floatx16 (&acc)[MI][2])
{
#pragma unroll
    for (int mi = 0; mi < MI; ++mi)
#pragma unroll
        for (int ni = 0; ni < 2; ++ni)
#pragma unroll
            for (int bm = 0; bm < 2; ++bm)
            {
                floatx4 x = acc4[2 * mi + bm][2 * ni], y = acc4[2 * mi + bm][2 * ni + 1];
                gp_k32_to_square(x, y);
#pragma unroll
                for (int j = 0; j < 4; ++j)
                {
                    acc[mi][ni][8 * bm + j] = x[j];
                    acc[mi][ni][8 * bm + 4 + j] = y[j];
                }
            }
}

__device__ __forceinline__ void split2_f16(const float (&x)[8], float scale, uint4 &p1, uint4 &p2)
{
    f16x8 h1, h2;
#pragma unroll
    for (int j = 0; j < 8; ++j)
    {
        const float v = x[j] * scale;
        h1[j] = (_Float16)v;
        h2[j] = (_Float16)(v - (float)h1[j]);
    }
    p1 = *reinterpret_cast<uint4 *>(&h1);
    p2 = *reinterpret_cast<uint4 *>(&h2);
}

template <int ITER> __global__ __launch_bounds__(256) void split_planes_kernel(SplitArgs a)
{
    const int tg = blockIdx.z, tid = threadIdx.x, lane = tid & 63;
    const int m = blockIdx.x * 4 + (tid >> 6);
    const float *src = a.src[tg] + (size_t)m * a.ld_src;
    unsigned short *dst = a.dst[tg] + (size_t)m * a.ld_dst + a.col0_dst;
    const float *sc = a.scale[tg], *mn = a.mean[tg];
    const bool adaptive = a.rowunscale[tg] != nullptr;
    const bool live = m < a.rows_valid && m % a.Tp < a.T;
    float xs[ITER][8];
    float sum = 0.f, mx = 0.f;
#pragma unroll
    for (int it = 0; it < ITER; ++it)
    {
        const int k = (it * 64 + lane) * 8;
#pragma unroll
        for (int j = 0; j < 8; ++j)
            xs[it][j] = 0.f;
        if (k < a.cols && live)
        {
            const float4 v0 = stream_load4(src + k), v1 = stream_load4(src + k + 4);
            xs[it][0] = v0.x; xs[it][1] = v0.y; xs[it][2] = v0.z; xs[it][3] = v0.w;
            xs[it][4] = v1.x; xs[it][5] = v1.y; xs[it][6] = v1.z; xs[it][7] = v1.w;
            if (sc)
#pragma unroll
                for (int j = 0; j < 8; ++j)
                    xs[it][j] = xs[it][j] * sc[k + j] + mn[k + j];
        }
        sum += ((xs[it][0] + xs[it][1]) + (xs[it][2] + xs[it][3])) + ((xs[it][4] + xs[it][5]) + (xs[it][6] + xs[it][7]));
#pragma unroll
        for (int j = 0; j < 8; ++j)
            mx = fmaxf(mx, fabsf(xs[it][j]));
    }
#pragma unroll
    for (int off = 32; off >= 1; off >>= 1)
    {
        sum += __shfl_xor(sum, off, 64);
        mx = fmaxf(mx, __shfl_xor(mx, off, 64));
    }
    float scale = (float)(1 << GP_SPLIT_FIXED_EXP), unscale = 1.0f / (float)(1 << GP_SPLIT_FIXED_EXP);
    if (adaptive)
    {
        int e = 0;
        if (mx > 0.f && mx < 3.0e38f)
        {
            int x;
            (void)frexpf(mx, &x);
            e = min(max(GP_SPLIT_FIXED_EXP + 1 - x, -100), 100);
        }
        scale = ldexpf(1.0f, e);
        unscale = ldexpf(1.0f, -e);
    }
    if (lane == 0)
    {
        if (a.rowsum[tg])
            a.rowsum[tg][m] = sum;
        if (adaptive)
            a.rowunscale[tg][m] = unscale;
    }
#pragma unroll
    for (int it = 0; it < ITER; ++it)
    {
        const int k = (it * 64 + lane) * 8;
        if (k < a.cols)
        {
            uint4 p1, p2;
            split2_f16(xs[it], scale, p1, p2);
            stream_store4u(reinterpret_cast<uint4 *>(dst + k), p1);
            stream_store4u(reinterpret_cast<uint4 *>(dst + a.plane + k), p2);
        }
    }
}

template <int ITER> __global__ __launch_bounds__(256) void split_planes_shared_kernel(SplitArgs a, int ntargets)
{
    const int tid = threadIdx.x, lane = tid & 63;
    const int m = blockIdx.x * 4 + (tid >> 6);
    const float *src = a.src[0] + (size_t)m * a.ld_src;
    const bool live = m < a.rows_valid && m % a.Tp < a.T;
    float x[ITER][8];
#pragma unroll
    for (int it = 0; it < ITER; ++it)
    {
        const int k = (it * 64 + lane) * 8;
#pragma unroll
        for (int j = 0; j < 8; ++j)
            x[it][j] = 0.f;
        if (k < a.cols && live)
        {
            const float4 v0 = stream_load4(src + k), v1 = stream_load4(src + k + 4);
            x[it][0] = v0.x; x[it][1] = v0.y; x[it][2] = v0.z; x[it][3] = v0.w;
            x[it][4] = v1.x; x[it][5] = v1.y; x[it][6] = v1.z; x[it][7] = v1.w;
        }
    }
    for (int tg = 0; tg < ntargets; ++tg)
    {
        unsigned short *dst = a.dst[tg] + (size_t)m * a.ld_dst + a.col0_dst;
        const float *sc = a.scale[tg], *mn = a.mean[tg];
        float xs[ITER][8];
        float sum = 0.f, mx = 0.f;
#pragma unroll
        for (int it = 0; it < ITER; ++it)
        {
            const int k = (it * 64 + lane) * 8;
#pragma unroll
            for (int j = 0; j < 8; ++j)
                xs[it][j] = 0.f;
            if (k < a.cols && live)
#pragma unroll
                for (int j = 0; j < 8; ++j)
                    xs[it][j] = x[it][j] * sc[k + j] + mn[k + j];
            sum += ((xs[it][0] + xs[it][1]) + (xs[it][2] + xs[it][3])) + ((xs[it][4] + xs[it][5]) + (xs[it][6] + xs[it][7]));
#pragma unroll
            for (int j = 0; j < 8; ++j)
                mx = fmaxf(mx, fabsf(xs[it][j]));
        }
#pragma unroll
        for (int off = 32; off >= 1; off >>= 1)
        {
            sum += __shfl_xor(sum, off, 64);
            mx = fmaxf(mx, __shfl_xor(mx, off, 64));
        }
        int e = 0;
        if (mx > 0.f && mx < 3.0e38f)
        {
            int xe;
            (void)frexpf(mx, &xe);
            e = min(max(GP_SPLIT_FIXED_EXP + 1 - xe, -100), 100);
        }
        const float scale = ldexpf(1.0f, e), unscale = ldexpf(1.0f, -e);
        if (lane == 0)
        {
            a.rowsum[tg][m] = sum;
            a.rowunscale[tg][m] = unscale;
        }
#pragma unroll
        for (int it = 0; it < ITER; ++it)
        {
            const int k = (it * 64 + lane) * 8;
            if (k < a.cols)
            {
                uint4 p1, p2;
                split2_f16(xs[it], scale, p1, p2);
                stream_store4u(reinterpret_cast<uint4 *>(dst + k), p1);
                stream_store4u(reinterpret_cast<uint4 *>(dst + a.plane + k), p2);
            }
        }
    }
}

template <int MODE, int NBP, int WM, int WN>
__global__ __launch_bounds__(64 * WM * WN, (WM * WN >= 16) ? 1 : 2) void gemm_planes_kernel(GemmPArgs args)
// ... 176 lines not shown
            }
            cur = cur == 2 ? 0 : cur + 1;
        }
        if (GP_PROFILE && blockIdx.x == 64 && blockIdx.z == 0 && (tid == 0 || tid == 64 * 7))
            printf("# gemm_planes<%d,%d> wave %d trips %d: cycles per trip  dma-issue %lld  fragments+mfma %lld  wait-dma %lld  barrier %lld\n", MODE, NBP,
                   wave, nk - 2, pf[0] / (nk - 2), pf[1] / (nk - 2), pf[2] / (nk - 2), pf[3] / (nk - 2));
        if (nk > 1)
        {
            GP_COMPUTE(cur)
            GP_WAIT(0);
            __syncthreads();
            cur = cur == 2 ? 0 : cur + 1;
        }
        GP_COMPUTE(cur)
    }
    else
    {
        for (int kt = 0; kt < nk - 1; ++kt)
        {
            const int cur = kt & 1;
            if (!GP_EXPERIMENT_NO_DMA)
                GP_DMA(cur ^ 1, (kt + 1) * GP_BK)
            if (!GP_EXPERIMENT_NO_MFMA)
                GP_COMPUTE(cur)
            GP_WAIT(0);
            __syncthreads();
        }
        GP_COMPUTE((nk - 1) & 1)
    }
#undef GP_WAIT
#undef GP_DMA
#undef GP_LD
#undef GP_TERM
#undef GP_COMPUTE
#if GP_MFMA_K32
    floatx16 acc[MI][2];
    gp_k32_to_squares<MI>(acc4, acc);
#else
#undef GP_MFMA
#endif
    {
        const int sel = n0 >= tg.bsplit ? 1 : 0;
        const float bsc = tg.bs[sel], o2 = tg.bo2[sel];
        float *const fx = reinterpret_cast<float *>(gp_smem);
        __syncthreads();
        for (int i = tid; i < BM; i += 64 * NW)
        {
            const int m = m0 + i;
            fx[i] = bsc * (tg.rsc ? tg.rsc[m] : args.a_unscale);
            fx[BM + i] = o2 * (tg.rs2 ? (tg.rs0[m] + tg.rs1[m]) + tg.rs2[m] : tg.rs1 ? tg.rs0[m] + tg.rs1[m] : tg.rs0[m]);
        }
        __syncthreads();
#pragma unroll
        for (int mi = 0; mi < MI; ++mi)
#pragma unroll
            for (int rq = 0; rq < 4; ++rq)
            {
                const int ml = wm * 32 * MI + mi * 32 + 8 * rq + 4 * lh;
                const float4 mu = *reinterpret_cast<const float4 *>(fx + ml), ad = *reinterpret_cast<const float4 *>(fx + BM + ml);
                const float mus[4] = {mu.x, mu.y, mu.z, mu.w}, ads[4] = {ad.x, ad.y, ad.z, ad.w};
#pragma unroll
                for (int j = 0; j < 4; ++j)
                {
                    const int r = 4 * rq + j;
                    acc[mi][0][r] = mus[j] * acc[mi][0][r] + ads[j];
                    acc[mi][1][r] = mus[j] * acc[mi][1][r] + ads[j];
                }
                asm volatile("" ::: "memory");
            }
    }
    GemmTarget et;
    et.C = tg.C;
    et.e0 = tg.e0; et.e1 = tg.e1; et.e2 = tg.e2; et.e3 = tg.e3;
    et.q0 = tg.q0; et.q1 = tg.q1;
    GemmArgs ea;
    ea.M = args.M;
    ea.ldc = args.ldc;
    ea.T = args.T;
    ea.Tp_lane = args.Tp_lane;
    ea.lanes = args.lanes;
    ea.mag_lane = args.mag_lane;
#pragma unroll
    for (int half = 0; half < MI / 2; ++half)
        gemm_epilogue<MODE>(et, ea, m0 + wm * 32 * MI + half * 64, n0, 0, wn, lr, lh, acc[2 * half][0], acc[2 * half][1], acc[2 * half + 1][0],
                            acc[2 * half + 1][1]);
}

}
```

umx.cpp_amd/csrc/gemm_planes_pp.h:

```cpp
#pragma once
#include "gemm_planes.h"

#ifndef PP_DMA_BOTH
#define PP_DMA_BOTH 1
#endif

namespace umx
{

template <int MODE, int NBP> __global__ __launch_bounds__(512, 1) void gemm_planes_pp_kernel(GemmPArgs args)
{
    extern __shared__ __attribute__((aligned(16))) unsigned char gp_smem[];
    constexpr int MI = 4, BM = 256, BN = 256;
    constexpr int A_PL = BM * 64, B_PL = BN * 64;
    constexpr int BUF_BYTES = 2 * A_PL + NBP * B_PL, STAGES = gp_stages(4, 4, NBP);
    [[maybe_unused]] constexpr int PH = 1, KKP = 2 / PH;
    static_assert(NBP == 1 || NBP == 2, "weight planes: 1 (u8) or 2 (u16, fp32)");
    const GemmPTarget tg = args.t[blockIdx.z];
    const int tid = threadIdx.x, lane = tid & 63, wave = __builtin_amdgcn_readfirstlane(tid >> 6);
    const int grp = wave >> 2, ws = wave & 3;
    const int wm = grp, wn = ws, lr = lane & 31, lh = lane >> 5;
    int tile_m, tile_n;
    {
        const int gx = args.N / BN, gy = args.M / BM, total = gx * gy;
// ... 182 lines not shown
                else
                    PP_WAIT_VM(0);
            }
            PP_BARRIER()
        }
        cur = cur + 1 == STAGES ? 0 : cur + 1;
    }
    if (grp == 0)
        PP_BARRIER()
    if (PP_PROFILE)
        pq[2] = clock64();
#undef PP_DMA
#undef PP_LD
#undef PP_LOAD
#if !GP_MFMA_K32
#undef PP_MFMA
#endif
#undef PP_TERM
#undef PP_MMA
#undef PP_WAIT_VM
#undef PP_WAIT_LDS
#undef PP_BARRIER
#if GP_MFMA_K32
    floatx16 acc[MI][2];
    gp_k32_to_squares<MI>(acc4, acc);
#endif
    {
        const int sel = n0 >= tg.bsplit ? 1 : 0;
        const float bsc = tg.bs[sel], o2 = tg.bo2[sel];
        float *const fx = reinterpret_cast<float *>(gp_smem);
        __syncthreads();
        for (int i = tid; i < BM; i += 512)
        {
            const int m = m0 + i;
            fx[i] = bsc * (tg.rsc ? tg.rsc[m] : args.a_unscale);
            fx[BM + i] = o2 * (tg.rs2 ? (tg.rs0[m] + tg.rs1[m]) + tg.rs2[m] : tg.rs1 ? tg.rs0[m] + tg.rs1[m] : tg.rs0[m]);
        }
        __syncthreads();
#pragma unroll
        for (int mi = 0; mi < MI; ++mi)
#pragma unroll
            for (int rq = 0; rq < 4; ++rq)
            {
                const int ml = wm * 32 * MI + mi * 32 + 8 * rq + 4 * lh;
                const float4 mu = *reinterpret_cast<const float4 *>(fx + ml), ad = *reinterpret_cast<const float4 *>(fx + BM + ml);
                const float mus[4] = {mu.x, mu.y, mu.z, mu.w}, ads[4] = {ad.x, ad.y, ad.z, ad.w};
#pragma unroll
                for (int j = 0; j < 4; ++j)
                {
                    const int r = 4 * rq + j;
                    acc[mi][0][r] = mus[j] * acc[mi][0][r] + ads[j];
                    acc[mi][1][r] = mus[j] * acc[mi][1][r] + ads[j];
                }
                asm volatile("" ::: "memory");
            }
    }
    if (PP_PROFILE)
        pq[3] = clock64();
    GemmTarget et;
    et.C = tg.C;
    et.e0 = tg.e0; et.e1 = tg.e1; et.e2 = tg.e2; et.e3 = tg.e3;
    et.q0 = tg.q0; et.q1 = tg.q1;
    GemmArgs ea;
    ea.M = args.M;
    ea.ldc = args.ldc;
    ea.T = args.T;
    ea.Tp_lane = args.Tp_lane;
    ea.lanes = args.lanes;
    ea.mag_lane = args.mag_lane;
    if (PP_EXPERIMENT & 8)
    {
        float s = 0.f;
#pragma unroll
        for (int mi = 0; mi < MI; ++mi)
#pragma unroll
            for (int r = 0; r < 16; ++r)
                s += acc[mi][0][r] + acc[mi][1][r];
        if (s == 12345.678f)
            tg.C[tid] = s;
        return;
    }
#pragma unroll
    for (int half = 0; half < MI / 2; ++half)
        gemm_epilogue<MODE>(et, ea, m0 + wm * 32 * MI + half * 64, n0, 0, wn, lr, lh, acc[2 * half][0], acc[2 * half][1], acc[2 * half + 1][0],
                            acc[2 * half + 1][1]);
    if (PP_PROFILE)
    {
        pq[4] = clock64();
        __builtin_amdgcn_s_waitcnt(0x0f70);
        pq[5] = clock64();
        if ((blockIdx.x == 264 || blockIdx.x == 2000) && blockIdx.z == 1 && (tid == 0 || tid == 64 * 4))
            printf("# pp<%d,%d> wg %d wave %d trips %d: cycles  first-tile-wait %lld  main-loop %lld (%lld per trip)  fix-up %lld  epilogue-issue %lld  store-drain %lld  total %lld\n",
                   MODE, NBP, (int)blockIdx.x, wave, nk, pq[1] - pq[0], pq[2] - pq[1], (pq[2] - pq[1]) / nk, pq[3] - pq[2], pq[4] - pq[3], pq[5] - pq[4], pq[5] - pq[0]);
    }
}

}
```

umx.cpp_amd/csrc/gemm_planes_ps.h:

```cpp
#pragma once
#include "gemm_planes_pp.h"

namespace umx
{

typedef unsigned int v4u32 __attribute__((ext_vector_type(4)));
constexpr int PS_TAB_ROWS = 4, PS_TAB_COLS = 8;
__host__ __device__ constexpr int ps_lds_bytes(int NBP) { return gp_lds_bytes(4, 4, NBP) + (PS_TAB_ROWS + PS_TAB_COLS) * 256 * 4; }
constexpr unsigned PS_DROP = 0x40000000u;
#ifndef PS_STORE_AUX
#define PS_STORE_AUX 2
#endif
#ifndef PS_PREWAIT
#define PS_PREWAIT 1
#endif
#ifndef PS_A_AUX
#define PS_A_AUX 0
#endif
#ifndef PS_B_AUX
#define PS_B_AUX 0
#endif
#ifndef PS_PROFILE
#define PS_PROFILE 0
#endif
// ... 187 lines not shown
            PS_TERM(0, NBP - 1, kl)                                                                                  \
        PS_TERM(0, 0, kl)                                                                                            \
    }
#endif
#define PS_WAIT_VM(n) __builtin_amdgcn_s_waitcnt(0x0f70 | ((n) & 15) | (((n) >> 4) << 14))
#define PS_WAIT_LDS() __builtin_amdgcn_s_waitcnt(0xc07f)
#define PS_BARRIER()                                                                                                 \
    {                                                                                                                \
        __builtin_amdgcn_sched_barrier(0);                                                                           \
        __builtin_amdgcn_s_barrier();                                                                                \
        __builtin_amdgcn_sched_barrier(0);                                                                           \
    }

    int e_m0 = 0, e_n0 = 0, e_tgi = 0, e_ln0 = 0, e_f0 = 0;
    __amdgpu_buffer_rsrc_t rsC = __builtin_amdgcn_make_buffer_rsrc(args.t[0].C, 0, 0, 0x00020000);
    const unsigned ldc4 = (unsigned)args.ldc * 4u;
    const float4 *const row4 = reinterpret_cast<const float4 *>(rowtab);
    const uint4 *const row4u = reinterpret_cast<const uint4 *>(rowtab);
    float cv[2][7];
    unsigned cvo[2];
    float4 nx_mu, nx_ad;
    uint4 nx_ro;
    int e_row = 0;
#define PS_EPI_ROWS(g_)                                                                                              \
    {                                                                                                                \
        nx_mu = row4[e_row + 2 * (g_)];                                                                              \
        nx_ad = row4[64 + e_row + 2 * (g_)];                                                                         \
        nx_ro = row4u[128 + e_row + 2 * (g_)];                                                                       \
    }
#define PS_EPI_SETUP()                                                                                               \
    {                                                                                                                \
        int el_ = lane;                                                                                              \
        asm volatile("" : "+v"(el_));                                                                                \
        e_row = wm * 32 + (el_ >> 5);                                                                                \
        _Pragma("unroll") for (int ni = 0; ni < 2; ++ni)                                                             \
        {                                                                                                            \
            const int cl_ = wn * 64 + ni * 32 + (el_ & 31);                                                          \
            cvo[ni] = (unsigned)cl_ * 4u;                                                                            \
            cv[ni][4] = coltab[4 * 256 + cl_];                                                                       \
            if (MODE != G_IH)                                                                                        \
            {                                                                                                        \
                cv[ni][0] = coltab[cl_];                                                                             \
                cv[ni][1] = coltab[256 + cl_];                                                                       \
                cv[ni][2] = coltab[2 * 256 + cl_];                                                                   \
                cv[ni][3] = coltab[3 * 256 + cl_];                                                                   \
            }                                                                                                        \
            if (MODE == G_FC3)                                                                                       \
            {                                                                                                        \
                cv[ni][5] = coltab[5 * 256 + cl_];                                                                   \
                cv[ni][6] = coltab[6 * 256 + cl_];                                                                   \
                cvo[ni] = reinterpret_cast<const unsigned *>(coltab)[7 * 256 + cl_];                                 \
            }                                                                                                        \
        }                                                                                                            \
        PS_EPI_ROWS(0)                                                                                               \
        if (MODE == G_FC3)                                                                                           \
        {                                                                                                            \
            const size_t lane_b_ = args.mag_lane * 4, all_b_ = (size_t)(args.lanes ? args.lanes : args.M / args.Tp_lane) * lane_b_; \
            const size_t lo_ = (size_t)e_ln0 * lane_b_, rest_ = all_b_ > lo_ ? all_b_ - lo_ : 0;                      \
            rsC = __builtin_amdgcn_make_buffer_rsrc(reinterpret_cast<unsigned char *>(args.t[e_tgi].C) + lo_, 0,     \
                                                    (int)(rest_ < 2 * lane_b_ ? rest_ : 2 * lane_b_), 0x00020000);   \
        }                                                                                                            \
        else                                                                                                         \
            rsC = __builtin_amdgcn_make_buffer_rsrc(args.t[e_tgi].C + ((size_t)e_m0 * args.ldc + e_n0), 0, 0x7fffffff, 0x00020000); \
    }
#define PS_EPI_BAND(mi)                                                                                              \
    _Pragma("unroll") for (int rq = 0; rq < 4; ++rq)                                                                 \
    {                                                                                                                \
        const float mus_[4] = {nx_mu.x, nx_mu.y, nx_mu.z, nx_mu.w}, ads_[4] = {nx_ad.x, nx_ad.y, nx_ad.z, nx_ad.w};  \
        const unsigned ro_[4] = {nx_ro.x, nx_ro.y, nx_ro.z, nx_ro.w};                                                \
        if ((mi)*4 + rq + 1 < 16)                                                                                    \
            PS_EPI_ROWS((mi)*4 + rq + 1)                                                                             \
        if ((rq & 1) == 0)                                                                                           \
        {                                                                                                            \
            PS_EPI_SWAP(mi, rq >> 1)                \
        }                                                                                                            \
        float ys_[2][4];                                                                                             \
        unsigned os_[2][4];                                                                                          \
        _Pragma("unroll") for (int ni = 0; ni < 2; ++ni)                                                             \
            _Pragma("unroll") for (int j = 0; j < 4; ++j)                                                            \
            {                                                                                                        \
                float y = mus_[j] * PS_ACC(mi, ni, 4 * rq + j) + ads_[j];                                            \
                if (MODE == G_IH)                                                                                    \
                    y = y + cv[ni][4];                                          \
                else                                                                                                 \
                {                                                                                                    \
                    y = div_by(y - cv[ni][0], cv[ni][1], cv[ni][2]) * cv[ni][3] + cv[ni][4];  \
                    if (MODE == G_FC1)                                                                               \
                        y = tanh_epi(y);                                                                             \
                    else if (MODE == G_FC2)                                                                          \
                        y = fmaxf(y, 0.f);                                                                           \
                    else                                                                                             \
                        y = fmaxf(y * cv[ni][5] + cv[ni][6], 0.f);              \
                }                                                                                                    \
                ys_[ni][j] = y;                                                                                      \
                os_[ni][j] = ro_[j] + cvo[ni];                                                                       \
            }                                                                                                        \
        __builtin_amdgcn_sched_barrier(0);  \
        _Pragma("unroll") for (int ni = 0; ni < 2; ++ni)                                                             \
            _Pragma("unroll") for (int j = 0; j < 4; ++j)                                                            \
                __builtin_amdgcn_raw_buffer_store_b32(__float_as_uint(ys_[ni][j]), rsC, os_[ni][j], 0, PS_STORE_AUX);   \
        __builtin_amdgcn_sched_barrier(0);                                                                           \
    }

    const unsigned lds_row = lds0 + STAGES * BUF_BYTES, lds_col = lds_row + PS_TAB_ROWS * 1024;
#define PS_TAB_PIECE(PTR, LDSOFF, FIRST_ELEM)                                                                        \
    {                                                                                                                \
        if (PTR)                                                                                                     \
            __builtin_amdgcn_raw_ptr_buffer_load_lds(__builtin_amdgcn_make_buffer_rsrc(const_cast<float *>(PTR), 0, 0x7fffffff, 0x00020000), \
                                                     (lds_ptr)(size_t)((LDSOFF) + ws * 256), 4, lane * 4, ((FIRST_ELEM) + ws * 64) * 4, 0, 0); \
    }
#define PS_TAB_RAW()                                                                                                 \
    {                                                                                                                \
        const GemmPTarget &tg_ = args.t[c_tgi];                                                                      \
        if (!BOTH || grp == 0)                                                                                       \
        {                                                                                                            \
            PS_TAB_PIECE(tg_.rsc, lds_row, c_m0)                                                                     \
            PS_TAB_PIECE(tg_.rs0, lds_row + 1024, c_m0)                                                              \
            PS_TAB_PIECE(tg_.rs1, lds_row + 2048, c_m0)                                                              \
            PS_TAB_PIECE(tg_.rs2, lds_row + 3072, c_m0)                                                              \
        }                                                                                                            \
        if (!BOTH || grp == 1)                                                                                       \
        {                                                                                                            \
            if (MODE == G_IH)                                                                                        \
                PS_TAB_PIECE(tg_.e0, lds_col + 4 * 1024, c_n0)                                                       \
            else                                                                                                     \
            {                                                                                                        \
                PS_TAB_PIECE(tg_.e0, lds_col, c_n0)                                                                  \
                PS_TAB_PIECE(tg_.e1, lds_col + 1024, c_n0)                                                           \
                PS_TAB_PIECE(tg_.e2, lds_col + 3 * 1024, c_n0)                                                       \
                PS_TAB_PIECE(tg_.e3, lds_col + 4 * 1024, c_n0)                                                       \
            }                                                                                                        \
            if (MODE == G_FC3)                                                                                       \
            {                                                                                                        \
                PS_TAB_PIECE(tg_.q0, lds_col + 5 * 1024, c_n0)                                                       \
                PS_TAB_PIECE(tg_.q1, lds_col + 6 * 1024, c_n0)                                                       \
            }                                                                                                        \
        }                                                                                                            \
    }
#define PS_TAB_FINISH()                                                                                              \
    {                                                                                                                \
        if (grp == 0)                                                                                                \
        {                                                                                                            \
            const GemmPTarget &tg_ = args.t[e_tgi];                                                                  \
            const int sel_ = e_n0 >= tg_.bsplit ? 1 : 0;                                                             \
            const float rsc_ = tg_.rsc ? rowtab[tid] : args.a_unscale, r0_ = rowtab[256 + tid];                      \
            const float r1_ = tg_.rs1 ? rowtab[512 + tid] : 0.f, r2_ = tg_.rs2 ? rowtab[768 + tid] : 0.f;            \
            unsigned off_ = (unsigned)tid * ldc4;                        \
            if (MODE == G_FC3)                                                                                       \
            {                                                                                                        \
                                                      \
                const int f1_ = e_f0 + tid, second_ = f1_ >= args.Tp_lane ? 1 : 0, f_ = f1_ - second_ * args.Tp_lane; \
                off_ = f_ < args.T ? ((unsigned)second_ * (unsigned)args.mag_lane + (unsigned)f_ * MAGP) * 4u : PS_DROP; \
            }                                                                                                        \
            rowtab[tid] = tg_.bs[sel_] * rsc_;                            \
            rowtab[256 + tid] = tg_.bo2[sel_] * (tg_.rs2 ? (r0_ + r1_) + r2_ : tg_.rs1 ? r0_ + r1_ : r0_);           \
            reinterpret_cast<unsigned *>(rowtab)[512 + tid] = off_;                                                  \
            if (MODE != G_IH)                                                                                        \
            {                                                                                                        \
                const float sd_ = sqrtf(coltab[256 + tid] + 1e-5f);                         \
                coltab[256 + tid] = sd_;                                                                             \
                coltab[2 * 256 + tid] = 1.0f / sd_;                                                                  \
            }                                                                                                        \
            if (MODE == G_FC3)                                                                                       \
            {                                                                                                        \
                          \
                const int n_ = e_n0 + tid, ch_ = n_ >= MAGP ? 1 : 0, bin_ = n_ - ch_ * MAGP;                         \
                reinterpret_cast<unsigned *>(coltab)[7 * 256 + tid] = bin_ < NBINS ? ((unsigned)(ch_ * args.T) * MAGP + (unsigned)bin_) * 4u : PS_DROP; \
            }                                                                                                        \
        }                                                                                                            \
    }

    int cur = 0, u = 0;
#define PS_M(FIRST, LATE, YOUNG1, TAB, FINISH, SPLIT)                                                                       \
    {                                                                                                                \
        const int nxt_ = STAGES == 3 ? (cur == 0 ? 2 : cur - 1) : cur ^ 1;  \
        const bool more_ = u + STAGES - 1 < ntrips, late_ = (LATE) && grp == 0;                                      \
        if ((TAB) && issuer)                                                                                         \
            PS_TAB_RAW()                                                                                             \
        if (more_ && !late_)                                                                                         \
        {                                                                                                            \
            if (issuer)                                                                                              \
                PS_DMA_ISSUE(nxt_)                                                                                   \
            PS_DMA_ADVANCE()                                                                                         \
        }                                                                                                            \
        PS_LOAD_KL(cur, 0)                                                                                           \
        if (!(FIRST))                                                                                                \
            PS_LOAD_KL(cur, 1)                                                                                       \
        if (FINISH)                                                                                                  \
            PS_TAB_FINISH()                                                                                          \
        PS_WAIT_LDS();                                                                                               \
        if (BOTH && grp == 1 && u + 1 < ntrips)                                                                      \
        {                                                                                                            \
             \
            if (YOUNG1)                                                                                              \
            {                                                                                                        \
                if (!PS_PREWAIT)                                                                                     \
                    PS_WAIT_VM(63);                                                                                  \
            }                                                                                                        \
            else if (u + 2 < ntrips)                                                                                 \
                PS_WAIT_VM(DMA_PER_WAVE);                                                                            \
            else                                                                                                     \
                PS_WAIT_VM(0);                                                                                       \
        }                                                                                                            \
        if (!(SPLIT) || grp == 0)              \
            PS_BARRIER()                                                                                             \
        if (more_ && late_)                                                                                          \
        {                                                                                                            \
            PS_DMA_ISSUE(nxt_)                                                                                       \
            PS_DMA_ADVANCE()                                                                                         \
        }                                                                                                            \
    }
#define PS_C_END(YOUNG0)                                                                                             \
    {                                                                                                                \
        if (grp == 0 && u + 1 < ntrips)                                                                              \
        {                                                                                                            \
            if (YOUNG0)                                                                                              \
            {                                                                                                        \
                if (!PS_PREWAIT)                                                                                     \
                    PS_WAIT_VM(63);                                                                                  \
            }                                                                                                        \
            else if (STAGES == 3 && u + 2 < ntrips)                                                                  \
                PS_WAIT_VM(DMA_PER_WAVE);                                                                            \
            else                                                                                                     \
                PS_WAIT_VM(0);                                                                                       \
        }                                                                                                            \
        PS_BARRIER()                                                                                                 \
        cur = cur + 1 == STAGES ? 0 : cur + 1;                                                                       \
        ++u;                                                                                                         \
    }
#define PS_C_FIRST_TAIL()                                                                                            \
    {                                                                                                                \
        PS_LOAD_KL(cur, 1)                                                                                           \
        PS_WAIT_LDS();                                                                                               \
        PS_STEP(1)                                                                                                   \
    }

    const int tab_trip = nk - 3;
    {
        if (issuer)
            PS_DMA_ISSUE(0)
        PS_DMA_ADVANCE()
        if (STAGES == 3)
        {
            if (issuer)
                PS_DMA_ISSUE(1)
            PS_DMA_ADVANCE()
            if (issuer)
                PS_WAIT_VM(DMA_PER_WAVE);
        }
        else if (issuer)
// ... 110 lines not shown
```

umx.cpp_amd/csrc/quant_planes.h:

```cpp
#pragma once
#include <cmath>
#include <cstddef>
#include <cstdint>
#include <cstring>

namespace umx
{

struct QuantCentre
{
    int c;
    float o2;
};
constexpr int QUANT_U8_MID = 128, QUANT_U8_CMIN = 0, QUANT_U8_CMAX = 255;
constexpr int QUANT_U16_MID = 32896, QUANT_U16_CMIN = 31, QUANT_U16_CMAX = 65504;
inline QuantCentre quant_centre(float s, float o, int elem_size = 1)
{
    const bool u16 = elem_size == 2;
    int c = u16 ? QUANT_U16_MID : QUANT_U8_MID;
    if (s - s == 0.f && s != 0.f && o - o == 0.f)
    {
        const double z = std::nearbyint(-(double)o / (double)s), lo = u16 ? QUANT_U16_CMIN : QUANT_U8_CMIN, hi = u16 ? QUANT_U16_CMAX : QUANT_U8_CMAX;
        c = (int)(z < lo ? lo : z > hi ? hi : z);
    }
    return {c, (float)((double)o + (double)c * (double)s)};
}

inline unsigned short f16_rne_bits(float f)
{
    unsigned u;
    memcpy(&u, &f, 4);
    const unsigned sign = (u >> 16) & 0x8000u;
    u &= 0x7fffffffu;
    if (u >= 0x7f800000u)
        return (unsigned short)(sign | 0x7c00u | (u > 0x7f800000u ? 0x200u : 0u));
    if (u >= 0x477ff000u)
        return (unsigned short)(sign | 0x7c00u);
    if (u < 0x38800000u)
    {
        if (u < 0x33000000u)
            return (unsigned short)sign;
        float a;
        memcpy(&a, &u, 4);
        const float scaled = a * 16777216.0f;
        const float r = nearbyintf(scaled);
        return (unsigned short)(sign | (unsigned)r);
    }
    const unsigned mant = u & 0x7fffffu, exp = (u >> 23) - 112u;
    unsigned h = (exp << 10) | (mant >> 13);
    const unsigned rem = mant & 0x1fffu;
    if (rem > 0x1000u || (rem == 0x1000u && (h & 1u)))
        ++h;
    return (unsigned short)(sign | h);
}
inline float f16_bits_to_float(unsigned short h)
{
    const unsigned sign = (unsigned)(h & 0x8000u) << 16, e = (h >> 10) & 31u, m = h & 0x3ffu;
    float v;
    if (e == 0)
        v = ldexpf((float)m, -24);
    else if (e == 31)
        v = m ? NAN : INFINITY;
    else
        v = ldexpf((float)(m | 0x400u), (int)e - 25);
    return sign ? -v : v;
}

inline void f16_split(float v, unsigned short *hi, unsigned short *lo)
{
    *hi = f16_rne_bits(v);
    if (lo)
        *lo = f16_rne_bits(v - f16_bits_to_float(*hi));
}

inline QuantCentre quant_planes(const void *q, int elem_size, int rows, int cols, const int *dst_row, size_t cols_pad, float s, float o,
                                unsigned short *hi, unsigned short *lo)
{
    const QuantCentre qc = quant_centre(s, o, elem_size);
    const unsigned char *q8 = static_cast<const unsigned char *>(q);
    for (int r = 0; r < rows; ++r)
    {
        const size_t d0 = (size_t)(dst_row ? dst_row[r] : r) * cols_pad, s0 = (size_t)r * cols;
        for (int k = 0; k < cols; ++k)
        {
            uint16_t qv = q8[s0 + k];
            if (elem_size == 2)
                memcpy(&qv, q8 + (s0 + k) * 2, 2);
            f16_split((float)((int)qv - qc.c), hi + d0 + k, elem_size == 2 ? lo + d0 + k : nullptr);
        }
    }
    return qc;
}

}
```

Before: 39520.

## Densify FC3 output columns to 4096 and compute Nyquist bins in split kernel

FC3 previously ran over a padded N (two channels of MAGP columns each) with dead padding columns. Now the planes GEMM runs on a dense N of 4096 (2048 bins per channel), and the two Nyquist-bin outputs are computed as dot products inside the activation split kernel that already streams each fc2 row. The split kernel also processes several rows per workgroup. This removes padded GEMM tiles and column-liveness checks, at the cost of extra per-row dot-product work and more complex weight and parameter layout.

```diff
diff --git a/include/umx_hip.h b/include/umx_hip.h
--- a/include/umx_hip.h
+++ b/include/umx_hip.h
@@ -293,6 +293,7 @@
 int umx_hip_debug_lstm_profile(umx_hip_ctx *ctx, unsigned long long *out48);
 int umx_hip_debug_lstm_placement(umx_hip_ctx *ctx, unsigned long long *out, int n);
 int umx_hip_debug_lds_guard(umx_hip_ctx *ctx, int launches, int rounds, unsigned *out2);
+int umx_hip_debug_fill_masks(umx_hip_ctx *ctx, float value);
 unsigned umx_hip_debug_f16_bits(float x);
 int umx_hip_debug_quant_centre(float scale, float offset, float *o2);
 int umx_hip_debug_quant_planes(const void *q, int elem_size, int n, float scale, float offset, unsigned short *hi, unsigned short *lo, float *o2);
diff --git a/umx.cpp_amd/__init__.py b/umx.cpp_amd/__init__.py
--- a/umx.cpp_amd/__init__.py
+++ b/umx.cpp_amd/__init__.py
@@ -244,6 +244,7 @@
                                                     C.c_int, C.c_void_p]
     lib.umx_hip_track_normalise_device.argtypes = [C.c_void_p, C.POINTER(C.c_void_p), C.c_void_p, C.c_int, C.c_void_p]
     lib.umx_hip_debug_lds_guard.argtypes = [C.c_void_p, C.c_int, C.c_int, C.POINTER(C.c_uint)]
+    lib.umx_hip_debug_fill_masks.argtypes = [C.c_void_p, C.c_float]
     lib.umx_hip_split_inference.argtypes = [C.c_void_p, _fp, C.c_int, C.POINTER(_fp), C.c_uint, C.c_void_p, C.c_void_p]
     lib.umx_hip_shift_inference.argtypes = [C.c_void_p, _fp, C.c_int, C.c_int, C.POINTER(_fp), C.c_uint, C.c_void_p,
                                             C.c_void_p]
@@ -356,7 +357,7 @@
                "umx_hip_lstm_was_persistent", "umx_hip_lstm_mode", "umx_hip_lstm_kernel_name", "umx_hip_gemm_kernel_name", "umx_hip_debug_wiener_bins", "umx_hip_debug_gate_math", "umx_hip_debug_lstm_profile", "umx_hip_debug_lstm_placement",
                "umx_hip_stream_layer_floats", "umx_hip_stream_get_layer", "umx_hip_stream_set_layer",
                "umx_hip_segment_begin", "umx_hip_segment_lstm_layer", "umx_hip_segment_end",
-               "umx_hip_split_inference", "umx_hip_shift_inference", "umx_hip_debug_lds_guard", "umx_hip_debug_f16_bits", "umx_hip_debug_quant_centre", "umx_hip_debug_quant_planes",
+               "umx_hip_split_inference", "umx_hip_shift_inference", "umx_hip_debug_lds_guard", "umx_hip_debug_fill_masks", "umx_hip_debug_f16_bits", "umx_hip_debug_quant_centre", "umx_hip_debug_quant_planes",
                "umx_hip_segment_masks_device", "umx_hip_target_mag_device", "umx_hip_segment_finish_device", "umx_hip_gate_reserve", "umx_hip_segment_discard", "umx_hip_pipeline_depth",
                "umx_hip_resampled_length", "umx_hip_resample_device", "umx_hip_shift_inference_rate", "umx_hip_separate_tracks_rate",
                "umx_hip_debug_resample_taps", "umx_hip_residual_slot", "umx_hip_segment_residual_device",
@@ -1170,7 +1171,12 @@
             return buf.reshape(T, H)
         if what == "mask":
             return buf.reshape(T, NOUT)
+        if what == "mask_raw":
+            return buf.reshape(2, T, -1)
         return buf
+
+    def debug_fill_masks(self, value):
+        self._check(self.lib.umx_hip_debug_fill_masks(self.h, C.c_float(value)))
 
     def stage_times(self, slot=None):
         names = (C.c_char_p * 32)()
diff --git a/umx.cpp_amd/csrc/engine.hip b/umx.cpp_amd/csrc/engine.hip
--- a/umx.cpp_amd/csrc/engine.hip
+++ b/umx.cpp_amd/csrc/engine.hip
@@ -74,6 +74,7 @@
     float *ih_b[3] = {};
     float *bn2[4] = {};
     float *bn3[4] = {}, *out_scale = nullptr, *out_mean = nullptr;
+    float *fc3_nyq = nullptr;
 };
 
 struct TargetAct
diff --git a/umx.cpp_amd/csrc/engine_cabi.h b/umx.cpp_amd/csrc/engine_cabi.h
--- a/umx.cpp_amd/csrc/engine_cabi.h
+++ b/umx.cpp_amd/csrc/engine_cabi.h
@@ -1008,6 +1008,21 @@
         ok = hipMemcpy(cell, dcell, no * 4, hipMemcpyDeviceToHost) == hipSuccess;
     (void)hipFree(d);
     return ok ? UMX_OK : UMX_ERR_HIP;
+}
+
+int umx_hip_debug_fill_masks(umx_hip_ctx *ctx, float value)
+{
+    if (!ctx)
+        return UMX_ERR_ARG;
+    if (int rc = ctx->sync_all())
+        return rc;
+    unsigned bits;
+    memcpy(&bits, &value, 4);
+    for (int si = 0; si < ctx->nslots; ++si)
+        for (int tg = 0; tg < 4; ++tg)
+            UMX_HIP_CHECK_CTX(ctx, hipMemsetD32(reinterpret_cast<hipDeviceptr_t>(ctx->slot[si].lane[0].ta[tg].mag), (int)bits, (size_t)ctx->B * 2 * ctx->T * MAGP));
+    UMX_HIP_CHECK_CTX(ctx, hipDeviceSynchronize());
+    return UMX_OK;
 }
 
 int umx_hip_debug_lds_guard(umx_hip_ctx *ctx, int launches, int rounds, unsigned *out2)
@@ -1371,6 +1386,7 @@
     else if (w == "proj") { src = sl.ta[target].P; nfl = (size_t)T * 4 * H; }
     else if (w == "fc2") { src = sl.ta[target].a2; nfl = (size_t)T * H; }
     else if (w == "mask") { src = sl.ta[target].mag; computed = 3; nfl = (size_t)T * NOUT; }
+    else if (w == "mask_raw") { src = sl.ta[target].mag; nfl = (size_t)2 * T * MAGP; }
     else if (w == "target_mag") { src = sl.ta[target].mag; computed = 2; nfl = (size_t)2 * T * NBINS; }
     else if (w == "y") { src = sl.y + (size_t)target * 2 * T * NBINS; nfl = (size_t)2 * 2 * T * NBINS; }
     else if (w == "max_abs") { src = sl.maxabs; nfl = 1; }
diff --git a/umx.cpp_amd/csrc/engine_init.h b/umx.cpp_amd/csrc/engine_init.h
--- a/umx.cpp_amd/csrc/engine_init.h
+++ b/umx.cpp_amd/csrc/engine_init.h
@@ -143,9 +143,14 @@
         for (int g = 0; g < 4; ++g)
             for (int u = 0; u < 16; ++u)
                 gate_row[g * Hl + sl * 16 + u] = sl * 64 + u * 4 + g;
+    const int fc3_n = gemm_planes ? FC3_N_PLANES : NOUT_PAD;
+    auto fc3_col = [&](int r) {
+        const int c = r / NBINS, bin = r % NBINS;
+        return !gemm_planes ? c * MAGP + bin : bin < FC3_BINS_PLANES ? c * FC3_BINS_PLANES + bin : -1;
+    };
     std::vector<int> fc3_row(NOUT);
     for (int r = 0; r < NOUT; ++r)
-        fc3_row[r] = r / NBINS * MAGP + r % NBINS;
+        fc3_row[r] = fc3_col(r);
     struct WeightDesc
     {
         std::string name[2];
@@ -159,7 +164,7 @@
         wd[W_IH0 + l] = {{"lstm.weight_ih_l" + std::to_string(l), "lstm.weight_ih_l" + std::to_string(l) + "_reverse"}, 2, G, H, G, H, &gate_row,
                          UMX_DTYPE_U8};
     wd[W_FC2] = {{"fc2.weight"}, 1, H, 2 * H, H, 2 * H, nullptr, UMX_DTYPE_U16};
-    wd[W_FC3] = {{"fc3.weight"}, 1, NOUT, H, NOUT_PAD, H, &fc3_row, UMX_DTYPE_U16};
+    wd[W_FC3] = {{"fc3.weight"}, 1, NOUT, H, fc3_n, H, &fc3_row, UMX_DTYPE_U16};
     auto upload_weight = [&](GemmWeight &w, const void *host, size_t bytes) -> int {
         unsigned char *p = nullptr;
         if (int rc = dalloc(&p, bytes, false))
@@ -200,7 +205,8 @@
             {
                 const umx_tensor_view *tv = view(tg, d.name[s]);
                 for (int r = 0; r < d.rows; ++r)
-                    memcpy(&qh[dst(s, r) * esz], static_cast<const unsigned char *>(tv->data) + (size_t)r * d.cols * esz, (size_t)d.cols * esz);
+                    if (!d.dst_row || (*d.dst_row)[r] >= 0)
+                        memcpy(&qh[dst(s, r) * esz], static_cast<const unsigned char *>(tv->data) + (size_t)r * d.cols * esz, (size_t)d.cols * esz);
                 w.s[s] = tv->scale;
                 w.o[s] = tv->offset;
             }
@@ -221,7 +227,8 @@
             if (!get(tg, d.name[s], (size_t)d.rows * d.cols, v))
                 return UMX_ERR_MODEL;
             for (int r = 0; r < d.rows; ++r)
-                memcpy(&f[dst(s, r)], &v[(size_t)r * d.cols], sizeof(float) * d.cols);
+                if (!d.dst_row || (*d.dst_row)[r] >= 0)
+                    memcpy(&f[dst(s, r)], &v[(size_t)r * d.cols], sizeof(float) * d.cols);
             if (gemm_planes)
             {
                 float mx = 0.f, scale = 1.f;
@@ -287,18 +294,26 @@
             return rc;
         if (!get(tg, "output_scale", NBINS, v))
             return UMX_ERR_MODEL;
-        w.assign(NOUT_PAD, 0.f);
-        for (int c = 0; c < 2; ++c)
-            for (int k = 0; k < NBINS; ++k)
-                w[c * MAGP + k] = v[k];
+        float nyq[2][SPLIT_NYQ_PARAMS] = {};
+        auto fc3_vector = [&](const std::vector<float> &per_row, float fill, int k) {
+            w.assign(fc3_n, fill);
+            for (int r = 0; r < NOUT; ++r)
+                if (fc3_col(r) >= 0)
+                    w[fc3_col(r)] = per_row[r];
+                else
+                    nyq[r / NBINS][k] = per_row[r];
+        };
+        std::vector<float> v2(NOUT);
+        for (int r = 0; r < NOUT; ++r)
+            v2[r] = v[r % NBINS];
+        fc3_vector(v2, 0.f, 4);
         if (int rc = upload(&b.out_scale, w))
             return rc;
         if (!get(tg, "output_mean", NBINS, v))
             return UMX_ERR_MODEL;
-        w.assign(NOUT_PAD, 0.f);
-        for (int c = 0; c < 2; ++c)
-            for (int k = 0; k < NBINS; ++k)
-                w[c * MAGP + k] = v[k];
+        for (int r = 0; r < NOUT; ++r)
+            v2[r] = v[r % NBINS];
+        fc3_vector(v2, 0.f, 5);
         if (int rc = upload(&b.out_mean, w))
             return rc;
         if (int rc = load_weight(tg, wd[W_FC1], b.w[W_FC1]))
@@ -316,11 +331,23 @@
                 return rc;
             if (!get(tg, std::string("bn3.") + bnn[k], NOUT, v))
                 return UMX_ERR_MODEL;
-            w.assign(NOUT_PAD, k == 1 ? 1.f : 0.f);
+            fc3_vector(v, k == 1 ? 1.f : 0.f, k);
+            if (int rc = upload(&b.bn3[k], w))
+                return rc;
+        }
+        if (gemm_planes)
+        {
+            if (!get(tg, "fc3.weight", (size_t)NOUT * H, v))
+                return UMX_ERR_MODEL;
+            w.assign((size_t)2 * H + 2 * SPLIT_NYQ_PARAMS, 0.f);
             for (int c = 0; c < 2; ++c)
-                memcpy(&w[c * MAGP], &v[c * NBINS], sizeof(float) * NBINS);
-            if (int rc = upload(&b.bn3[k], w))
-                return rc;
+            {
+                memcpy(&w[(size_t)c * H], &v[((size_t)c * NBINS + FC3_BINS_PLANES) * H], sizeof(float) * H);
+                memcpy(&w[(size_t)2 * H + c * SPLIT_NYQ_PARAMS], nyq[c], sizeof nyq[c]);
+            }
+            if (int rc = upload(&b.fc3_nyq, w))
+                return rc;
+            weight_bytes += w.size() * sizeof(float);
         }
         if (int rc = load_weight(tg, wd[W_FC2], b.w[W_FC2]))
             return rc;
diff --git a/umx.cpp_amd/csrc/engine_stages.h b/umx.cpp_amd/csrc/engine_stages.h
--- a/umx.cpp_amd/csrc/engine_stages.h
+++ b/umx.cpp_amd/csrc/engine_stages.h
@@ -89,6 +89,7 @@
         default:
             a.src[i] = c.a2; a.dst[i] = c.a2_p; a.rowsum[i] = c.rs_a2; a.rowunscale[i] = c.rsc_a2;
             a.cols = H; a.ld_src = H; a.ld_dst = H; a.col0_dst = 0; a.plane = rows_all * H;
+            a.nyq[i] = b.fc3_nyq; a.mask[i] = c.mag; a.mag_lane = (size_t)2 * T * MAGP;
             break;
         }
     }
@@ -97,6 +98,15 @@
     if (which == SP_XS && a.cols <= 3072)
     {
         hipLaunchKernelGGL(split_planes_shared_kernel<6>, dim3(grid.x), dim3(256), 0, st, a, nact);
+        return;
+    }
+    if (which == SP_A2)
+    {
+        const dim3 grid_nyq(grid.x / SPLIT_NYQ_ROWS, 1, nact);
+        if (a.cols <= 1024)
+            hipLaunchKernelGGL((split_planes_kernel<2, true>), grid_nyq, dim3(256), 0, st, a);
+        else
+            hipLaunchKernelGGL((split_planes_kernel<4, true>), grid_nyq, dim3(256), 0, st, a);
         return;
     }
     if (a.cols <= 1024)
@@ -154,7 +164,7 @@
             t.A = c.a2_p; t.C = c.mag; t.rs0 = c.rs_a2; t.rsc = c.rsc_a2;
             t.e0 = b.bn3[0]; t.e1 = b.bn3[1]; t.e2 = b.bn3[2]; t.e3 = b.bn3[3];
             t.q0 = b.out_scale; t.q1 = b.out_mean;
-            g.N = NOUT_PAD; g.K = H; g.lda = H; g.ldc = 0; g.a_plane = rows_all * H;
+            g.N = FC3_N_PLANES; g.K = H; g.lda = H; g.ldc = 0; g.a_plane = rows_all * H;
             break;
         }
         t.B = static_cast<const unsigned short *>(w.p);
diff --git a/umx.cpp_amd/csrc/gemm_common.h b/umx.cpp_amd/csrc/gemm_common.h
--- a/umx.cpp_amd/csrc/gemm_common.h
+++ b/umx.cpp_amd/csrc/gemm_common.h
@@ -16,6 +16,11 @@
     G_FC2 = 2,
     G_FC3 = 3
 };
+
+constexpr int FC3_N_PLANES = 4096, FC3_BINS_PLANES = 2048;
+template <bool DENSE> __host__ __device__ __forceinline__ int fc3_col_channel(int n) { return DENSE ? n >> 11 : (n >= MAGP ? 1 : 0); }
+template <bool DENSE> __host__ __device__ __forceinline__ int fc3_col_bin(int n) { return DENSE ? n & (FC3_BINS_PLANES - 1) : n - fc3_col_channel<false>(n) * MAGP; }
+template <bool DENSE> __host__ __device__ __forceinline__ bool fc3_col_live(int n) { return DENSE || fc3_col_bin<false>(n) < NBINS; }
 
 struct GemmTarget
 {
@@ -62,7 +67,13 @@
     return copysignf(ax < 0.5f ? small : big, x);
 }
 
-template <int MODE>
+__device__ __forceinline__ float fc3_mask_value(float y, float rm, float sd, float rsd, float gw, float gb, float osc, float omn)
+{
+    y = div_by(y - rm, sd, rsd) * gw + gb;
+    return fmaxf(y * osc + omn, 0.f);
+}
+
+template <int MODE, bool DENSE = false>
 __device__ __forceinline__ void gemm_epilogue(const GemmTarget &tg, const GemmArgs &args, int m0, int n0, int wm, int wn,
                                               int lr, int lh, const floatx16 &acc00, const floatx16 &acc01,
                                               const floatx16 &acc10, const floatx16 &acc11)
@@ -104,9 +115,8 @@
         {
             osc = tg.q0[n];
             omn = tg.q1[n];
-            const int c = n >= MAGP ? 1 : 0, bin = n - c * MAGP;
-            col = lo + (unsigned)(c * args.T) * MAGP + (unsigned)bin;
-            col_ok = bin < NBINS;
+            col = lo + (unsigned)(fc3_col_channel<DENSE>(n) * args.T) * MAGP + (unsigned)fc3_col_bin<DENSE>(n);
+            col_ok = fc3_col_live<DENSE>(n);
         }
         unsigned run = (col + (unsigned)fA * MAGP) * 4u;
         int frow = fB;
@@ -125,23 +135,23 @@
                     float y = mi == 0 ? (ni == 0 ? acc00[r] : acc01[r]) : (ni == 0 ? acc10[r] : acc11[r]);
                     if (MODE == G_IH)
                         tg.C[(size_t)(m0 + ml) * args.ldc + n] = y + gb;
+                    else if (MODE == G_FC3)
+                    {
+                        const bool second = frow >= 0;
+                        const int f = second ? frow : frow + tpl;
+                        const bool ok = col_ok && f < args.T;
+                        ys[j] = fc3_mask_value(y, rm, sd, rsd, gw, gb, osc, omn);
+                        offs[j] = ok ? run + (second ? dA : 0u) : 0xfffffff0u;
+                        run += MAGP * 4;
+                        frow += 1;
+                    }
                     else
                     {
                         y = div_by(y - rm, sd, rsd) * gw + gb;
                         if (MODE == G_FC1)
                             tg.C[(size_t)(m0 + ml) * args.ldc + n] = tanh_epi(y);
-                        else if (MODE == G_FC2)
+                        else
                             tg.C[(size_t)(m0 + ml) * args.ldc + n] = fmaxf(y, 0.f);
-                        else
-                        {
-                            const bool second = frow >= 0;
-                            const int f = second ? frow : frow + tpl;
-                            const bool ok = col_ok && f < args.T;
-                            ys[j] = fmaxf(y * osc + omn, 0.f);
-                            offs[j] = ok ? run + (second ? dA : 0u) : 0xfffffff0u;
-                            run += MAGP * 4;
-                            frow += 1;
-                        }
                     }
                 }
                 if (MODE == G_FC3)
diff --git a/umx.cpp_amd/csrc/gemm_planes.h b/umx.cpp_amd/csrc/gemm_planes.h
--- a/umx.cpp_amd/csrc/gemm_planes.h
+++ b/umx.cpp_amd/csrc/gemm_planes.h
@@ -49,7 +49,15 @@
     int T, Tp, cols, ld_src, ld_dst, col0_dst;
     int rows_valid;
     size_t plane;
+    const float *nyq[4];
+    float *mask[4];
+    size_t mag_lane;
 };
+constexpr int SPLIT_NYQ_PARAMS = 8;
+#ifndef SPLIT_NYQ_ROWS
+#define SPLIT_NYQ_ROWS 4
+#endif
+static_assert(64 % SPLIT_NYQ_ROWS == 0, "a launch's rows (a multiple of 256) in whole workgroups of 4 x SPLIT_NYQ_ROWS");
 
 typedef _Float16 f16x8 __attribute__((ext_vector_type(8)));
 
@@ -107,75 +115,120 @@
     p2 = *reinterpret_cast<uint4 *>(&h2);
 }
 
-template <int ITER> __global__ __launch_bounds__(256) void split_planes_kernel(SplitArgs a)
-{
+template <int ITER, bool NYQ = false> __global__ __launch_bounds__(256) void split_planes_kernel(SplitArgs a)
+{
+    constexpr int ROWS = NYQ ? SPLIT_NYQ_ROWS : 1;
     const int tg = blockIdx.z, tid = threadIdx.x, lane = tid & 63;
-    const int m = blockIdx.x * 4 + (tid >> 6);
-    const float *src = a.src[tg] + (size_t)m * a.ld_src;
-    unsigned short *dst = a.dst[tg] + (size_t)m * a.ld_dst + a.col0_dst;
     const float *sc = a.scale[tg], *mn = a.mean[tg];
     const bool adaptive = a.rowunscale[tg] != nullptr;
-    const bool live = m < a.rows_valid && m % a.Tp < a.T;
-    float xs[ITER][8];
-    float sum = 0.f, mx = 0.f;
-#pragma unroll
-    for (int it = 0; it < ITER; ++it)
-    {
-        const int k = (it * 64 + lane) * 8;
-#pragma unroll
-        for (int j = 0; j < 8; ++j)
-            xs[it][j] = 0.f;
-        if (k < a.cols && live)
-        {
-            const float4 v0 = stream_load4(src + k), v1 = stream_load4(src + k + 4);
-            xs[it][0] = v0.x; xs[it][1] = v0.y; xs[it][2] = v0.z; xs[it][3] = v0.w;
-            xs[it][4] = v1.x; xs[it][5] = v1.y; xs[it][6] = v1.z; xs[it][7] = v1.w;
-            if (sc)
+    [[maybe_unused]] float wq[2][ITER][8];
+    if (NYQ)
+#pragma unroll
+        for (int c = 0; c < 2; ++c)
+#pragma unroll
+            for (int it = 0; it < ITER; ++it)
+            {
+                const int k = (it * 64 + lane) * 8;
 #pragma unroll
                 for (int j = 0; j < 8; ++j)
-                    xs[it][j] = xs[it][j] * sc[k + j] + mn[k + j];
-        }
-        sum += ((xs[it][0] + xs[it][1]) + (xs[it][2] + xs[it][3])) + ((xs[it][4] + xs[it][5]) + (xs[it][6] + xs[it][7]));
-#pragma unroll
-        for (int j = 0; j < 8; ++j)
-            mx = fmaxf(mx, fabsf(xs[it][j]));
-    }
-#pragma unroll
-    for (int off = 32; off >= 1; off >>= 1)
-    {
-        sum += __shfl_xor(sum, off, 64);
-        mx = fmaxf(mx, __shfl_xor(mx, off, 64));
-    }
-    float scale = (float)(1 << GP_SPLIT_FIXED_EXP), unscale = 1.0f / (float)(1 << GP_SPLIT_FIXED_EXP);
-    if (adaptive)
-    {
-        int e = 0;
-        if (mx > 0.f && mx < 3.0e38f)
-        {
-            int x;
-            (void)frexpf(mx, &x);
-            e = min(max(GP_SPLIT_FIXED_EXP + 1 - x, -100), 100);
-        }
-        scale = ldexpf(1.0f, e);
-        unscale = ldexpf(1.0f, -e);
-    }
-    if (lane == 0)
-    {
-        if (a.rowsum[tg])
-            a.rowsum[tg][m] = sum;
+                    wq[c][it][j] = 0.f;
+                if (k < a.cols)
+                {
+                    const float4 w0 = *reinterpret_cast<const float4 *>(a.nyq[tg] + (size_t)c * a.cols + k);
+                    const float4 w1 = *reinterpret_cast<const float4 *>(a.nyq[tg] + (size_t)c * a.cols + k + 4);
+                    wq[c][it][0] = w0.x; wq[c][it][1] = w0.y; wq[c][it][2] = w0.z; wq[c][it][3] = w0.w;
+                    wq[c][it][4] = w1.x; wq[c][it][5] = w1.y; wq[c][it][6] = w1.z; wq[c][it][7] = w1.w;
+                }
+            }
+#pragma unroll 1
+    for (int r = 0; r < ROWS; ++r)
+    {
+        const int m = (blockIdx.x * 4 + (tid >> 6)) * ROWS + r;
+        const float *src = a.src[tg] + (size_t)m * a.ld_src;
+        unsigned short *dst = a.dst[tg] + (size_t)m * a.ld_dst + a.col0_dst;
+        const bool live = m < a.rows_valid && m % a.Tp < a.T;
+        float xs[ITER][8];
+        float sum = 0.f, mx = 0.f;
+        [[maybe_unused]] float dot0 = 0.f, dot1 = 0.f;
+#pragma unroll
+        for (int it = 0; it < ITER; ++it)
+        {
+            const int k = (it * 64 + lane) * 8;
+#pragma unroll
+            for (int j = 0; j < 8; ++j)
+                xs[it][j] = 0.f;
+            if (k < a.cols && live)
+            {
+                const float4 v0 = stream_load4(src + k), v1 = stream_load4(src + k + 4);
+                xs[it][0] = v0.x; xs[it][1] = v0.y; xs[it][2] = v0.z; xs[it][3] = v0.w;
+                xs[it][4] = v1.x; xs[it][5] = v1.y; xs[it][6] = v1.z; xs[it][7] = v1.w;
+                if (sc)
+#pragma unroll
+                    for (int j = 0; j < 8; ++j)
+                        xs[it][j] = xs[it][j] * sc[k + j] + mn[k + j];
+            }
+            sum += ((xs[it][0] + xs[it][1]) + (xs[it][2] + xs[it][3])) + ((xs[it][4] + xs[it][5]) + (xs[it][6] + xs[it][7]));
+#pragma unroll
+            for (int j = 0; j < 8; ++j)
+                mx = fmaxf(mx, fabsf(xs[it][j]));
+            if (NYQ)
+#pragma unroll
+                for (int j = 0; j < 8; ++j)
+                {
+                    dot0 = fmaf(xs[it][j], wq[0][it][j], dot0);
+                    dot1 = fmaf(xs[it][j], wq[1][it][j], dot1);
+                }
+        }
+#pragma unroll
+        for (int off = 32; off >= 1; off >>= 1)
+        {
+            sum += __shfl_xor(sum, off, 64);
+            mx = fmaxf(mx, __shfl_xor(mx, off, 64));
+            if (NYQ)
+            {
+                dot0 += __shfl_xor(dot0, off, 64);
+                dot1 += __shfl_xor(dot1, off, 64);
+            }
+        }
+        if (NYQ && live && lane < 2)
+        {
+            const float *pr = a.nyq[tg] + (size_t)2 * a.cols + lane * SPLIT_NYQ_PARAMS;
+            const float sd = sqrtf(pr[1] + 1e-5f);
+            const int ln = m / a.Tp, f = m - ln * a.Tp;
+            a.mask[tg][(size_t)ln * a.mag_lane + mask_index(lane, a.T, f, FC3_BINS_PLANES)] =
+                fc3_mask_value(lane ? dot1 : dot0, pr[0], sd, 1.0f / sd, pr[2], pr[3], pr[4], pr[5]);
+        }
+        float scale = (float)(1 << GP_SPLIT_FIXED_EXP), unscale = 1.0f / (float)(1 << GP_SPLIT_FIXED_EXP);
         if (adaptive)
-            a.rowunscale[tg][m] = unscale;
-    }
-#pragma unroll
-    for (int it = 0; it < ITER; ++it)
-    {
-        const int k = (it * 64 + lane) * 8;
-        if (k < a.cols)
-        {
-            uint4 p1, p2;
-            split2_f16(xs[it], scale, p1, p2);
-            stream_store4u(reinterpret_cast<uint4 *>(dst + k), p1);
-            stream_store4u(reinterpret_cast<uint4 *>(dst + a.plane + k), p2);
+        {
+            int e = 0;
+            if (mx > 0.f && mx < 3.0e38f)
+            {
+                int x;
+                (void)frexpf(mx, &x);
+                e = min(max(GP_SPLIT_FIXED_EXP + 1 - x, -100), 100);
+            }
+            scale = ldexpf(1.0f, e);
+            unscale = ldexpf(1.0f, -e);
+        }
+        if (lane == 0)
+        {
+            if (a.rowsum[tg])
+                a.rowsum[tg][m] = sum;
+            if (adaptive)
+                a.rowunscale[tg][m] = unscale;
+        }
+#pragma unroll
+        for (int it = 0; it < ITER; ++it)
+        {
+            const int k = (it * 64 + lane) * 8;
+            if (k < a.cols)
+            {
+                uint4 p1, p2;
+                split2_f16(xs[it], scale, p1, p2);
+                stream_store4u(reinterpret_cast<uint4 *>(dst + k), p1);
+                stream_store4u(reinterpret_cast<uint4 *>(dst + a.plane + k), p2);
+            }
         }
     }
 }
@@ -518,7 +571,7 @@
     ea.mag_lane = args.mag_lane;
 #pragma unroll
     for (int half = 0; half < MI / 2; ++half)
-        gemm_epilogue<MODE>(et, ea, m0 + wm * 32 * MI + half * 64, n0, 0, wn, lr, lh, acc[2 * half][0], acc[2 * half][1], acc[2 * half + 1][0],
+        gemm_epilogue<MODE, true>(et, ea, m0 + wm * 32 * MI + half * 64, n0, 0, wn, lr, lh, acc[2 * half][0], acc[2 * half][1], acc[2 * half + 1][0],
                             acc[2 * half + 1][1]);
 }
 
diff --git a/umx.cpp_amd/csrc/gemm_planes_pp.h b/umx.cpp_amd/csrc/gemm_planes_pp.h
--- a/umx.cpp_amd/csrc/gemm_planes_pp.h
+++ b/umx.cpp_amd/csrc/gemm_planes_pp.h
@@ -288,7 +288,7 @@
     }
 #pragma unroll
     for (int half = 0; half < MI / 2; ++half)
-        gemm_epilogue<MODE>(et, ea, m0 + wm * 32 * MI + half * 64, n0, 0, wn, lr, lh, acc[2 * half][0], acc[2 * half][1], acc[2 * half + 1][0],
+        gemm_epilogue<MODE, true>(et, ea, m0 + wm * 32 * MI + half * 64, n0, 0, wn, lr, lh, acc[2 * half][0], acc[2 * half][1], acc[2 * half + 1][0],
                             acc[2 * half + 1][1]);
     if (PP_PROFILE)
     {
diff --git a/umx.cpp_amd/csrc/gemm_planes_ps.h b/umx.cpp_amd/csrc/gemm_planes_ps.h
--- a/umx.cpp_amd/csrc/gemm_planes_ps.h
+++ b/umx.cpp_amd/csrc/gemm_planes_ps.h
@@ -293,15 +293,12 @@
                 float y = mus_[j] * PS_ACC(mi, ni, 4 * rq + j) + ads_[j];                                            \
                 if (MODE == G_IH)                                                                                    \
                     y = y + cv[ni][4];                                          \
+                else if (MODE == G_FC3)                                                                              \
+                    y = fc3_mask_value(y, cv[ni][0], cv[ni][1], cv[ni][2], cv[ni][3], cv[ni][4], cv[ni][5], cv[ni][6]); \
                 else                                                                                                 \
                 {                                                                                                    \
                     y = div_by(y - cv[ni][0], cv[ni][1], cv[ni][2]) * cv[ni][3] + cv[ni][4];  \
-                    if (MODE == G_FC1)                                                                               \
-                        y = tanh_epi(y);                                                                             \
-                    else if (MODE == G_FC2)                                                                          \
-                        y = fmaxf(y, 0.f);                                                                           \
-                    else                                                                                             \
-                        y = fmaxf(y * cv[ni][5] + cv[ni][6], 0.f);              \
+                    y = MODE == G_FC1 ? tanh_epi(y) : fmaxf(y, 0.f);                                                 \
                 }                                                                                                    \
                 ys_[ni][j] = y;                                                                                      \
                 os_[ni][j] = ro_[j] + cvo[ni];                                                                       \
@@ -374,9 +371,9 @@
             }                                                                                                        \
             if (MODE == G_FC3)                                                                                       \
             {                                                                                                        \
-                          \
-                const int n_ = e_n0 + tid, ch_ = n_ >= MAGP ? 1 : 0, bin_ = n_ - ch_ * MAGP;                         \
-                reinterpret_cast<unsigned *>(coltab)[7 * 256 + tid] = bin_ < NBINS ? ((unsigned)(ch_ * args.T) * MAGP + (unsigned)bin_) * 4u : PS_DROP; \
+                 \
+                const int n_ = e_n0 + tid;                                                                           \
+                reinterpret_cast<unsigned *>(coltab)[7 * 256 + tid] = ((unsigned)(fc3_col_channel<true>(n_) * args.T) * MAGP + (unsigned)fc3_col_bin<true>(n_)) * 4u; \
             }                                                                                                        \
         }                                                                                                            \
     }
diff --git a/umx.cpp_amd/csrc/quant_planes.h b/umx.cpp_amd/csrc/quant_planes.h
--- a/umx.cpp_amd/csrc/quant_planes.h
+++ b/umx.cpp_amd/csrc/quant_planes.h
@@ -80,6 +80,8 @@
     const unsigned char *q8 = static_cast<const unsigned char *>(q);
     for (int r = 0; r < rows; ++r)
     {
+        if (dst_row && dst_row[r] < 0)
+            continue;
         const size_t d0 = (size_t)(dst_row ? dst_row[r] : r) * cols_pad, s0 = (size_t)r * cols;
         for (int k = 0; k < cols; ++k)
         {
```

New measurement: 39730 (median of 6 runs). Within noise of the previous version (+0.5%).
